# boyden/NuHTC

Measured on AMD Instinct MI355X. Metric: tiles/sec (256x256) whole-node, higher is better.
Workload: dtype f32

## Files before the change

include/nuhtc_hip.h:

```cpp
#ifndef NUHTC_HIP_H
#define NUHTC_HIP_H

#include <stddef.h>
#include <stdint.h>

#ifdef __cplusplus
extern "C" {
#endif

#define NUHTC_ABI_VERSION 12

enum {
  NUHTC_OK = 0,
  NUHTC_E_INVALID = -1,
  NUHTC_E_HIP = -2,
  NUHTC_E_STATE = -3,
  NUHTC_E_CAPACITY = -4,
  NUHTC_E_NOTFOUND = -5
};

enum { NUHTC_CH_AS_IS = 0, NUHTC_CH_SWAP = 1 };

enum { NUHTC_PIPE_BF16_SPLIT = 0, NUHTC_PIPE_FP32 = 1 };

// ... 70 lines not shown
  NUHTC_OVERLAP_POLYGON = 1
};

int nuhtc_merge_overlap(int device, const int32_t* boxes, const float* scores, const int32_t* areas, const uint32_t* bits,
                        const int64_t* bit_off, int64_t n, int64_t n_words, int overlap, double thr, int x_min, int y_min,
                        int x_max, int y_max, uint8_t* keep_dev, void* stream);

int nuhtc_check(nuhtc_engine* e, void* stream);

int nuhtc_get_buffer(nuhtc_engine* e, const char* name, void** dev_ptr, int64_t* shape, int* ndim, int* dtype);

int nuhtc_op_gemm(nuhtc_engine* e, const float* A, const float* W, const float* bias, float* C, int M, int N, int K,
                  int act, void* stream);
int nuhtc_op_gemm_split(nuhtc_engine* e, const float* A, const float* W_dev, const float* W_host, const float* bias, float* C, int M,
                        int N, int K, int act, void* stream);
int nuhtc_op_ln_gemm(nuhtc_engine* e, const float* X_dev, int T, const int* rows_dev, const float* W_host, const float* bias_host, const float* ln_g_host,
                     const float* ln_b_host, float* C_dev, int M, int N, int K, int act, void* stream);
int nuhtc_op_gemm_ln_gemm(nuhtc_engine* e, const float* A_dev, const float* Wp_host, const float* bp_host, const float* res_dev, const int* row_map_dev,
                          const float* W_host, const float* bias_host, const float* ln_g_host, const float* ln_b_host, float* Y_dev, float* C_dev, int M,
                          int Kp, int K, int N, int act, void* stream);
int nuhtc_op_merge_ln_gemm(nuhtc_engine* e, const float* X_dev, int B, int H, int W, int C, const float* W_host, const float* ln_g_host,
                           const float* ln_b_host, float* Y_dev, void* stream);
int nuhtc_op_swin_mlp(nuhtc_engine* e, const float* x_dev, const float* ln_g_dev, const float* ln_b_dev, const float* w1_host,
                      const float* b1_dev, const float* w2_host, const float* b2_dev, float* out_dev, int T, int C, void* stream);
int nuhtc_op_swin_proj_mlp(nuhtc_engine* e, const float* x_dev, const float* att_dev, const float* wp_host, const float* bp_dev,
                           const float* ln_g_dev, const float* ln_b_dev, const float* w1_host, const float* b1_dev, const float* w2_host,
                           const float* b2_dev, float* out_dev, int T, int C, void* stream);
int nuhtc_op_roi_align(nuhtc_engine* e, const float* feat_nhwc, int N, int H, int W, const float* rois, int R, int P,
                       float spatial_scale, int sampling_ratio, float* out, void* stream);
int nuhtc_op_nms(nuhtc_engine* e, const float* boxes, const float* scores, int n, float iou_thr, int32_t* keep_idx,
                 int32_t* count_dev, void* stream);
int nuhtc_op_cc_mask(nuhtc_engine* e, const float* sem_pred_dev, int B, int h, int w, int H, int W, uint8_t* mask_out_dev, void* stream);
int nuhtc_op_cc_proposals(nuhtc_engine* e, const uint8_t* mask_dev, int B, int H, int W, int open, int min_area, int cap, uint8_t* opened_out,
                          uint8_t* filled_out, int32_t* labels_out, int32_t* stats_out, float* boxes_out, int32_t* counts_out,
                          int32_t* overflow_out, void* stream);
typedef struct nuhtc_conv3_args {
  const float* in;
  float* out;
  const float* w;
  const float* bias;
  int32_t nimg, H, W, act;
  const int32_t* nimg_dev;
  int32_t pipe;
  int32_t N2;
  const float* w2;
  const float* b2;
  int32_t act2, store_out;
  float* out2;
  const float* res2;
  float* out3;
  const float* wn1;
  const float* bn1;
  float* outn1;
  int32_t n_more;
  const float* more_in[3];
  float* more_out2[3];
  int32_t more_H[3], more_W[3];
} nuhtc_conv3_args;
int nuhtc_op_conv3(nuhtc_engine* e, const nuhtc_conv3_args* a, void* stream);
enum { NUHTC_ORDER_TOKEN = 0, NUHTC_ORDER_COMPACT = 1 };
typedef struct nuhtc_wmsa_args {
  const float* x;
  float* out;
  const float* ln_g;
  const float* ln_b;
  const float* qkv_w;
  const float* qkv_b;
  const float* rel_table;
  int32_t B, H, W, C;
  int32_t shifted, pipe, out_order;
} nuhtc_wmsa_args;
int nuhtc_op_window_msa(nuhtc_engine* e, const nuhtc_wmsa_args* a, void* stream);
int nuhtc_op_patch_embed(nuhtc_engine* e, const uint8_t* tiles_dev, int B, int th, int tw, int valid_h, int valid_w, float scale_factor, int channel_mode,
                         const float* mean, const float* std, const float* w_host, const float* b_host, const float* ln_g_host, const float* ln_b_host,
                         float* tok_dev, float* img_dev, void* stream);
int nuhtc_op_layernorm(nuhtc_engine* e, const float* x_dev, const float* g_dev, const float* b_dev, float* y_dev, int rows, int C, void* stream);
int nuhtc_op_merge_ln(nuhtc_engine* e, const float* x_dev, const float* g_dev, const float* b_dev, float* y_dev, int B, int H, int W, int C, void* stream);
int nuhtc_op_fpn_lateral(nuhtc_engine* e, const float* X_dev, int B, int H, int W, int C, const float* W_host, const float* bias_host, const float* ln_g_host,
                         const float* ln_b_host, const float* parent_dev, float* out_dev, void* stream);
int nuhtc_op_sem_fuse(nuhtc_engine* e, const float* g0, const float* g1, const float* g2, const float* g3, float* out, int B, int H, int W, void* stream);
int nuhtc_op_pointwise64(nuhtc_engine* e, const float* x_dev, const float* w_dev, const float* b_dev, float* y_dev, int rows, const int32_t* rows_dev,
                         int rows_mul, int sigmoid, void* stream);
int nuhtc_op_fpn_mean_pool(nuhtc_engine* e, const float* const maps[4], const int32_t hw[4], int B, float* feat_dev, void* stream);
typedef struct nuhtc_bbox_tail_args {
  const float* h;
  const float* cls_w;
  const float* cls_b;
  const float* reg_w;
  const float* reg_b;
  int32_t nc, cap, refine;
  float stds[4];
  float img_w, img_h;
  const int32_t* r_dev;
  float* rois;
  float* cls;
  float* reg;
} nuhtc_bbox_tail_args;
int nuhtc_op_bbox_tail(nuhtc_engine* e, const nuhtc_bbox_tail_args* a, void* stream);
typedef struct nuhtc_det_post_args {
  const float* rois;
  const float* cls0;
  const float* cls1;
  const float* cls2;
  const float* reg2;
  const int32_t* roi_off;
  const int32_t* roi_cnt;
  int32_t B, nc, total, cap;
  float stds[4];
  float img_w, img_h, scale, score_thr, nms_iou;
  int32_t max_per_img, limit;
  float* dets;
  int32_t* labels;
  int32_t* counts;
  float* mask_rois;
  int32_t* det_off;
  int32_t* det_total;
  int32_t* cand_count;
  float* cand_scores;
  int32_t* cand_ids;
  float* cand_boxes;
} nuhtc_det_post_args;
int nuhtc_op_det_post(nuhtc_engine* e, const nuhtc_det_post_args* a, void* stream);
typedef struct nuhtc_paste_args {
  const float* prob;
  const float* mask_rois;
  const int32_t* det_off;
  const int32_t* det_counts;
  int32_t B, D, max_keep, H, W, vH, vW;
  float scale, thr;
  uint32_t* masks;
  int32_t* areas;
} nuhtc_paste_args;
int nuhtc_op_paste(nuhtc_engine* e, const nuhtc_paste_args* a, void* stream);
typedef struct nuhtc_tile_post_args {
  const float* dets;
  const int32_t* labels;
  const int32_t* areas;
  const int32_t* det_counts;
  const uint32_t* masks;
  uint8_t* keep;
  int32_t B, max_keep, H, W, vH, vW, margin, min_area;
  float thr;
} nuhtc_tile_post_args;
int nuhtc_op_tile_post(nuhtc_engine* e, const nuhtc_tile_post_args* a, void* stream);
int nuhtc_op_rpn_select(nuhtc_engine* e, const float* const out[4], const int32_t h[4], const int32_t w[4], int B, int nms_pre, int img_h, int img_w,
                        float min_size, float* cand_boxes, float* cand_scores, int32_t* cand_count, void* stream);
int nuhtc_op_nms_levels(nuhtc_engine* e, const float* boxes, const float* scores, const int32_t* group_count, int B, int G, int slot, float iou_thr,
                        int max_keep, int route, float* dets, int32_t* src, int32_t* counts, void* stream);
int nuhtc_op_build_rois(nuhtc_engine* e, const float* cc_boxes, const int32_t* cc_counts, int cc_cap, const float* rpn_dets, const int32_t* rpn_counts,
                        int rpn_cap, const float* fixed, int n_fixed, int B, int cap, float* rois, int32_t* roi_off, int32_t* roi_cnt, int32_t* total,
                        void* stream);

#define NUHTC_AP_AUTO 0
#define NUHTC_AP_GEMM 1
#define NUHTC_AP_KERNEL 2
#define NUHTC_AP_FP16 3
int nuhtc_op_attn_pool(nuhtc_engine* e, const float* F, int B, int HW, float tau, int route, float* G, void* stream);
typedef struct nuhtc_roi_feats_args {
  const float* x0;
  const float* x1;
  const float* sem;
  const float* x0sem;
  const float* G2;
  const float* G3;
  const float* rois;
  const int32_t* r_dev;
// ... 175 lines not shown
```

nuhtc_amd/csrc/common.h:

```cpp
#pragma once
#include <hip/hip_runtime.h>

#include <cstdint>
#include <cstdio>
#include <map>
#include <string>
#include <vector>

#include "../../include/nuhtc_hip.h"

#define WS 7
#define WS2 49
#define HEAD_DIM 32
#define FPN_C 64
#define FC_C 256

struct HostTensor {
  std::vector<float> data;
  std::vector<int64_t> shape;
};

struct BufInfo {
  void* ptr;
  std::vector<int64_t> shape;
  int dtype;
};

struct EngineError {
  int code;
  std::string msg;
};

#define HIP_CHECK(e, expr)                                                                              \
  do {                                                                                                  \
    hipError_t _err = (expr);                                                                           \
    if (_err != hipSuccess) {                                                                           \
      (e)->err = std::string(#expr) + " failed: " + hipGetErrorString(_err) + " at " + __FILE__ + ":" + \
                 std::to_string(__LINE__);                                                              \
      return NUHTC_E_HIP;                                                                               \
    }                                                                                                   \
  } while (0)

#define FAIL(e, code, message) \
  do {                         \
    (e)->err = (message);      \
    return (code);             \
  } while (0)

static inline int cdiv(int a, int b) { return (a + b - 1) / b; }
static inline bool launched() { return hipGetLastError() == hipSuccess; }

class DevScratch {
 public:
  DevScratch() = default;
  DevScratch(const DevScratch&) = delete;
  DevScratch& operator=(const DevScratch&) = delete;
  ~DevScratch() {
    for (void* p : ptrs_) hipFree(p);
  }
  template <typename T = void>
  T* alloc(size_t bytes) {
    void* p = nullptr;
    if (hipMalloc(&p, bytes) != hipSuccess) { ok_ = false; return nullptr; }
    ptrs_.push_back(p);
    return static_cast<T*>(p);
  }
  template <typename T>
  T* upload(const T* host, size_t n) {
    T* d = alloc<T>(n * sizeof(T));
    if (d && hipMemcpy(d, host, n * sizeof(T), hipMemcpyHostToDevice) != hipSuccess) { ok_ = false; return nullptr; }
    return d;
  }
  template <typename T>
  T* upload(const std::vector<T>& v) { return upload(v.data(), v.size()); }
  bool ok() const { return ok_; }

 private:
  std::vector<void*> ptrs_;
  bool ok_ = true;
};

struct ProfScope {
  ProfScope(const char* tag, double flops, double bytes, hipStream_t s);
  ~ProfScope();
  void device_rows(const int* m_dev, int m_mul, int m_cap);
  hipStream_t s_;
  int idx_;
};
bool prof_enabled();
int dev_knob(const char* name, int dflt);
int& dev_knob_ref(const char* name, int dflt);
#define DEV_SKIP(bit)                                    \
  do {                                                   \
    static const int& skip_ = dev_knob_ref("SKIP", 0);   \
    if (skip_ & (bit)) return 0;                         \
  } while (0)

enum AMode { A_PLAIN = 0, A_CONV3 = 1, A_LN = 2  };
enum Act { ACT_NONE = 0, ACT_RELU = 1, ACT_GELU = 2, ACT_COS = 3  };
enum StoreMode { ST_PLAIN = 0, ST_ROWMAP = 1, ST_DECONV2 = 2 };

struct Conv3Fuse {
  int N2;
  const void* w2f;
  const float* bias2;
  float* out2;
  int act2;
  const float* res2;
  float* out3;
  const float* wn1;
  const float* bn1;
  float* outn1;
  int store_out;
  int n_more;
  const float* more_in[3];
  float* more_out2[3];
  int more_H[3], more_W[3];
};
int conv3_pack_fuse(const float* w2_host, int N2, std::vector<unsigned short>& out);

struct GemmParams {
  const float* A;
  const float* W;
  const void* Wsplit;
  const float* bias;
  float* C;
  int M, N, K;
  int lda, ldc;
  const int* m_dev;
  int m_mul;
  int amode;
  const float* ln_part;
  int ln_nparts;
  const int* a_rows;
  int seg_k, seg_rows;
  const int* pad_rows;
  int n_pad;
  const float* pad_val;
  float* stats_out;
  int cH, cW, cC;
  const float* zeros;
  int act;
  float alpha;
  const float* res;
  int ldr;
  const float* up;
  int upH, upW;
  const int* row_map;
  int store;
  const float* cos_ri;
  const float* cos_rj;
  float cos_tau;
  int batch;
  long long sA, sW, sC, sRi, sRj;
  unsigned long long* stamps;
  int row_fastest;
  int throughput;
  const Conv3Fuse* fuse;
};
int launch_gemm(const GemmParams& p, hipStream_t s);
int gemm_make_split(const float* w_host, int N, int K, std::vector<unsigned short>& out);

bool conv3_split_supported(const GemmParams& p);
int launch_conv3_split(const GemmParams& p, hipStream_t s);

bool mlp_supported(int C);
size_t mlp_stream_bytes(int C);
void mlp_pack_stream(const float* w1, const float* w2, int C, std::vector<unsigned short>& out);
size_t proj_stream_bytes(int C);
void proj_pack_stream(const float* w, int C, std::vector<unsigned short>& out);
int launch_swin_mlp(const float* x_in, float* x_out, const float* ln_g, const float* ln_b, const void* wstream, const float* b1, const float* b2,
                    int T, int C, hipStream_t s, const float* att = nullptr, const void* pstream = nullptr, const float* bp = nullptr,
                    float* stats_out = nullptr );

bool lnqkv_supported(int C);
void lnqkv_pack_stream(const float* w, int C, std::vector<unsigned short>& out);
int launch_swin_lnqkv(const float* x, float* qkv, const int* src_tok, const int* dst_row, const int* pad_rows, int n_pad, const float* ln_g, const float* ln_b,
                      const void* wstream, const float* bias, int T, int C, hipStream_t s);

int launch_contours(const uint32_t* masks, const uint8_t* keep, const int32_t* counts, int B, int max_per_img, int H, int W,
                    int cap, int16_t* xy, int32_t* n, hipStream_t s);

struct ExportParams {
  const float* boxes; const int32_t* labels; const int32_t* counts; const uint8_t* keep; const uint32_t* masks;
  const int32_t* contour_n; const int16_t* contour_xy;
  int B, K, words, ccap, cap;
  int32_t* n_out; int64_t* idx; float* boxes_out; int32_t* labels_out; int32_t* cn_out; int16_t* xy_out; uint32_t* words_out;
};
int launch_export_kept(const ExportParams& p, int32_t* pos_scratch, hipStream_t s);
int launch_export_crops(const uint32_t* words, const int32_t* n_dev, int cap, int H, int wpr, int32_t* box, int32_t* area, int32_t* off, int32_t* size_scratch,
                        uint32_t* pool, int pool_cap, hipStream_t s);

void cv_linear_tables(int ssize, int dsize, bool horizontal, std::vector<int>& tab);
int launch_preproc(const uint8_t* tiles, float* img, int B, int th, int tw, int Hn, int Wn, int Hv, int Wv, const int* xtab, const int* ytab, int swap,
                   const float* mean_istd, hipStream_t s);
int launch_patch_embed_tiles(const uint8_t* tiles, int B, int th, int tw, int Hn, int Wn, int Hv, int Wv, const int* xtab, const int* ytab, int swap,
                             const float* mean_istd, const float* w, const float* b, const float* g, const float* beta, float* tok, hipStream_t s);
int launch_layernorm(const float* x, const int* src_map, const float* g, const float* b, float* y, int rows, int C, hipStream_t s);
int launch_ln_stats(const float* x, float* stats, int rows, int C, hipStream_t s);
int launch_layernorm_windows(const float* x, const int* src_map, const int* dst_map, const float* g, const float* b, float* y,
                             float* pad_dst, const float* pad_val, int rows, int C, hipStream_t s);
int launch_merge_ln(const float* x, const float* g, const float* b, float* y, int B, int H, int W, int C, hipStream_t s);
int launch_window_attn(const float* qkv, const float* biasP, const float* maskP, const int* mask_any, const int* out_map, float* out,
                       int nWinTotal, int nWperImg, int C, int nH, int split_pipe , hipStream_t s,
                       const unsigned long long* padbits = nullptr ,
                       int bias_row = 0);

int launch_sem_fuse(const float* g0, const float* g1, const float* g2, const float* g3, float* out, int B, int H, int W,
                    hipStream_t s);
int launch_conv1x1_n1(const float* x, const float* w, const float* b, float* y, int rows, int C, hipStream_t s);
int launch_rownorm_inv(const float* x, float* inv, int rows, int C, hipStream_t s);
int launch_transpose(const float* x, float* y, int batch, int rows, int cols, hipStream_t s);

#define POOL_CHUNK 256
struct PoolLevels { const float* x[4]; int hw[4]; int choff[5]; };
int pool_chunks(const int hw[4], int choff[5]);
int launch_fpn_mean_pool(const PoolLevels& p, int B, double* slab, float* feat, hipStream_t s);

int launch_roi_align(const float* feat, int N, int H, int W, int C, const float* rois, int R, const int* r_dev, int P,
                     float scale, int sr, float* out, int accumulate, hipStream_t s);

const char* nuhtc_tu_probe_conv();
const char* nuhtc_tu_probe_gemm();
const char* nuhtc_tu_probe_mlp();
const char* nuhtc_tu_probe_swin();
```

nuhtc_amd/csrc/dense.hip:

```cpp
#include "common.h"

__device__ __forceinline__ float4 bilin_ac(const float* __restrict__ g, int b, int h, int w, int y, int x, int H, int W, int c4) {
  const float sy = h > 1 ? (float)(h - 1) / (float)(H - 1) : 0.f;
  const float sx = w > 1 ? (float)(w - 1) / (float)(W - 1) : 0.f;
  const float fy = sy * y, fx = sx * x;
  const int y0 = (int)fy, x0 = (int)fx;
  const int y1 = y0 + (y0 < h - 1 ? 1 : 0), x1 = x0 + (x0 < w - 1 ? 1 : 0);
  const float ly = fy - y0, lx = fx - x0, hy = 1.f - ly, hx = 1.f - lx;
  const float4* p = reinterpret_cast<const float4*>(g) + (long long)b * h * w * 16 + c4;
  const float4 v00 = p[(y0 * w + x0) * 16], v01 = p[(y0 * w + x1) * 16], v10 = p[(y1 * w + x0) * 16], v11 = p[(y1 * w + x1) * 16];
  float4 r;
  r.x = hy * (hx * v00.x + lx * v01.x) + ly * (hx * v10.x + lx * v11.x);
  r.y = hy * (hx * v00.y + lx * v01.y) + ly * (hx * v10.y + lx * v11.y);
  r.z = hy * (hx * v00.z + lx * v01.z) + ly * (hx * v10.z + lx * v11.z);
  r.w = hy * (hx * v00.w + lx * v01.w) + ly * (hx * v10.w + lx * v11.w);
  return r;
}

__global__ void sem_fuse_kernel(const float* __restrict__ g0, const float* __restrict__ g1, const float* __restrict__ g2,
                                const float* __restrict__ g3, float* __restrict__ out, int B, int H, int W) {
  long long idx = (long long)blockIdx.x * blockDim.x + threadIdx.x;
  long long total = (long long)B * H * W * 16;
  if (idx >= total) return;
  int c4 = idx & 15;
  long long pix = idx >> 4;
  int x = pix % W, y = (pix / W) % H, b = pix / ((long long)W * H);
  float4 a = reinterpret_cast<const float4*>(g0)[idx];
  float4 r = make_float4(fmaxf(a.x, 0.f), fmaxf(a.y, 0.f), fmaxf(a.z, 0.f), fmaxf(a.w, 0.f));
  const float* gs[3] = {g1, g2, g3};
#pragma unroll
  for (int i = 0; i < 3; ++i) {
    int h = H >> (i + 1), w = W >> (i + 1);
    float4 u = bilin_ac(gs[i], b, h, w, y, x, H, W, c4);
    r.x += fmaxf(u.x, 0.f); r.y += fmaxf(u.y, 0.f); r.z += fmaxf(u.z, 0.f); r.w += fmaxf(u.w, 0.f);
  }
  reinterpret_cast<float4*>(out)[idx] = r;
}

int launch_sem_fuse(const float* g0, const float* g1, const float* g2, const float* g3, float* out, int B, int H, int W,
                    hipStream_t s) {
  ProfScope ps("sem_fuse", 0, 4.0 * 64 * B * H * W * 2.33, s);
  long long total = (long long)B * H * W * 16;
  hipLaunchKernelGGL(sem_fuse_kernel, dim3((unsigned)((total + 255) / 256)), dim3(256), 0, s, g0, g1, g2, g3, out, B, H, W);
  return launched() ? 0 : NUHTC_E_HIP;
}

__global__ void conv1x1_n1_kernel(const float* __restrict__ x, const float* __restrict__ w, const float* __restrict__ b,
                                  float* __restrict__ y, long long rows, const int* __restrict__ rows_dev, int rows_mul, int sigmoid) {
  if (rows_dev) { long long rd = (long long)(*rows_dev) * rows_mul; rows = rd < rows ? rd : rows; }
  const int l = threadIdx.x & 15;
  const float4 ww = reinterpret_cast<const float4*>(w)[l];
  const float bias = b[0];
  const long long stride = ((long long)gridDim.x * blockDim.x) >> 4;
  for (long long row = ((long long)blockIdx.x * blockDim.x + threadIdx.x) >> 4; row < rows; row += stride) {
    const float4 v = reinterpret_cast<const float4*>(x)[row * 16 + l];
    float acc = v.x * ww.x + v.y * ww.y + v.z * ww.z + v.w * ww.w;
    acc += __shfl_xor(acc, 1); acc += __shfl_xor(acc, 2); acc += __shfl_xor(acc, 4); acc += __shfl_xor(acc, 8);
    if (l == 0) {
      const float u = acc + bias;
      y[row] = sigmoid ? 1.0f / (1.0f + expf(-u)) : u;
    }
  }
}

int launch_conv1x1_n1(const float* x, const float* w, const float* b, float* y, int rows, int C, hipStream_t s) {
  if (C != 64) return NUHTC_E_INVALID;
  long long threads = (long long)rows * 16;
  if (rows <= 0) return 0;
  hipLaunchKernelGGL(conv1x1_n1_kernel, dim3((unsigned)((threads + 255) / 256)), dim3(256), 0, s, x, w, b, y, (long long)rows,
                     (const int*)nullptr, 1, 0);
  return launched() ? 0 : NUHTC_E_HIP;
}

int launch_conv1x1_n1_dev(const float* x, const float* w, const float* b, float* y, int rows_cap, const int* rows_dev, int rows_mul,
                          int sigmoid, hipStream_t s) {
  long long threads = (long long)rows_cap * 16;
  if (rows_cap <= 0) return 0;
  const long long nb = (threads + 255) / 256;
  hipLaunchKernelGGL(conv1x1_n1_kernel, dim3((unsigned)(nb < 8192 ? nb : 8192)), dim3(256), 0, s, x, w, b, y, (long long)rows_cap,
                     rows_dev, rows_mul, sigmoid);
  return launched() ? 0 : NUHTC_E_HIP;
}

__global__ void rownorm_inv_kernel(const float* __restrict__ x, float* __restrict__ inv, long long rows) {
  long long row = ((long long)blockIdx.x * blockDim.x + threadIdx.x) >> 4;
  const int l = threadIdx.x & 15;
  float acc = 0.f;
  if (row < rows) {
    float4 v = reinterpret_cast<const float4*>(x)[row * 16 + l];
    acc = v.x * v.x + v.y * v.y + v.z * v.z + v.w * v.w;
  }
  acc += __shfl_xor(acc, 1); acc += __shfl_xor(acc, 2); acc += __shfl_xor(acc, 4); acc += __shfl_xor(acc, 8);
  if (row < rows && l == 0) inv[row] = 1.0f / fmaxf(sqrtf(acc), 1e-8f);
}

int launch_rownorm_inv(const float* x, float* inv, int rows, int C, hipStream_t s) {
  if (C != 64) return NUHTC_E_INVALID;
  long long threads = (long long)rows * 16;
  hipLaunchKernelGGL(rownorm_inv_kernel, dim3((unsigned)((threads + 255) / 256)), dim3(256), 0, s, x, inv, (long long)rows);
  return launched() ? 0 : NUHTC_E_HIP;
}

__global__ void transpose_kernel(const float* __restrict__ x, float* __restrict__ y, int rows, int cols) {
  __shared__ float t[32][33];
  const float* xb = x + (long long)blockIdx.z * rows * cols;
  float* yb = y + (long long)blockIdx.z * rows * cols;
  int c0 = blockIdx.x * 32, r0 = blockIdx.y * 32;
  int tx = threadIdx.x & 31, ty = threadIdx.x >> 5;
  for (int j = ty; j < 32; j += 8) {
    int r = r0 + j, c = c0 + tx;
    t[j][tx] = (r < rows && c < cols) ? xb[(long long)r * cols + c] : 0.f;
  }
  __syncthreads();
  for (int j = ty; j < 32; j += 8) {
    int c = c0 + j, r = r0 + tx;
    if (r < rows && c < cols) yb[(long long)c * rows + r] = t[tx][j];
  }
}

int launch_transpose(const float* x, float* y, int batch, int rows, int cols, hipStream_t s) {
  hipLaunchKernelGGL(transpose_kernel, dim3(cdiv(cols, 32), cdiv(rows, 32), batch), dim3(256), 0, s, x, y, rows, cols);
  return launched() ? 0 : NUHTC_E_HIP;
}
```

nuhtc_amd/csrc/engine.h:

```cpp
#pragma once
#include <unordered_map>

#include "common.h"

struct StageGeom {
  int H, W, C, nH;
  int Hp, Wp, nW;
  int* map[2];
  int* cidx[2];
  int* ctok[2];
  int* vrow[2];
  unsigned long long* padbits[2];
  int* brow;
  int bias_row;
  float* mask;
  int* mask_any;
};

enum BlockRoute { ROUTE_PLAIN, ROUTE_A_LN, ROUTE_FUSED };

struct BlockW {
  BlockRoute route;
  float *n1g, *n1b, *relbT , *qkv_w, *qkv_b, *proj_w, *proj_b, *n2g, *n2b, *f1_w, *f1_b, *f2_w, *f2_b;
  float *qkv_wln, *qkv_bln, *f1_wln, *f1_bln;
  void* qkv_stream;
  void* mlp_stream;
  void* proj_stream;
};

struct nuhtc_engine {
  nuhtc_config cfg;
  int device = 0;
  std::string err;
  std::map<std::string, HostTensor> raw;
  std::map<std::string, std::vector<int64_t>> schema;
  std::map<std::string, BufInfo> bufs;
  std::vector<void*> allocs;
  struct WSplit { const void* planes; int N, K; };
  std::unordered_map<const float*, WSplit> wsplit;
  bool finalized = false;
  bool debug_tokens = false;
  int lastB = 0;
  int Hn = 0, Wn = 0;
  int Hv = 0, Wv = 0;
  int vh = 0, vw = 0;
  int *rs_xtab = nullptr, *rs_ytab = nullptr;

  StageGeom st[4];
  float *pe_w = nullptr, *pe_b = nullptr, *pe_g = nullptr, *pe_beta = nullptr;
  std::vector<BlockW> blocks[4];
  bool merge_one_launch[3] = {}, out_ln_folded = false, conv_fuse = false;
  float *on_g[4], *on_b[4], *mg_g[3], *mg_b[3], *mg_w[3];
  float *mg_wln[3] = {}, *mg_bln[3] = {};
  int* mg_src[3] = {};
  float *lat_w[4], *lat_b[4], *fpn_w[4], *fpn_b[4];
  float *rpn_w, *rpn_b, *rpn_hw, *rpn_hb;
  void *rpn_hf, *sem_lf[4], *sem_ef;
  float *sem_lw[4], *sem_lb[4], *sem_cw[4], *sem_cb[4], *sem_ew, *sem_eb, *sem_gw, *sem_gb;
  float *fc1_w[3], *fc1_b[3], *fc2_w[3], *fc2_b[3], *head_w[3], *head_b[3];
  float *mk_w[4], *mk_b[4], *mk_up_w, *mk_up_b, *mk_lw, *mk_lb;

  float *img, *tokA, *tokB, *xw, *qkv, *att, *hid;
  float* tok[4] = {};
  float* ln_out[4] = {};
  float *lat_wln[4] = {}, *lat_bln[4] = {};
  const uint8_t* in_tiles = nullptr;
  int in_swap = 0;
  int last_batch = 0;
  float* ln_part2 = nullptr;
  float* ln_part = nullptr;
  float *c[4], *lat[4], *x[4], *rpn[4], *semg[4];
  float *tmpA, *tmpB, *tmpR, *sem_feat, *sem_pred, *x0sem;
  PoolLevels pool{};
  double* pool_slab = nullptr;
  int roi_cap = 0;
  int cand_cap = 0;
  int* overflow = nullptr;
  int* overflow_host = nullptr;
  int32_t* export_pos = nullptr;
  int32_t* crop_size = nullptr;
  hipStream_t own = nullptr;
  hipStream_t side = nullptr;
  hipEvent_t ev_rpn = nullptr, ev_side = nullptr, ev_fpn = nullptr;
  hipStream_t side2 = nullptr;
  hipEvent_t ev_side2 = nullptr;
  struct RoiWs* rw = nullptr;
};

int dev_alloc(nuhtc_engine* e, void** p, size_t bytes);
int upload_bytes(nuhtc_engine* e, void** dst, const void* host, size_t bytes);
template <typename T>
int upload(nuhtc_engine* e, T** dst, const std::vector<T>& v) {
  return upload_bytes(e, (void**)dst, v.data(), v.size() * sizeof(T));
}
template <typename T>
int ws(nuhtc_engine* e, T** p, const char* name, std::vector<int64_t> shape, int dtype) {
  size_t n = 1;
  for (auto d : shape) n *= (size_t)d;
  int rc = dev_alloc(e, (void**)p, n * sizeof(T));
  if (rc) return rc;
  if (name) e->bufs[name] = BufInfo{(void*)*p, shape, dtype};
  return 0;
}
const HostTensor* raw(nuhtc_engine* e, const std::string& name, std::initializer_list<int64_t> shape);
#define RAW(var, name, ...)                                 \
  const HostTensor* var = raw(e, (name), {__VA_ARGS__});    \
  if (!var) return NUHTC_E_STATE;
std::vector<float> pack_conv3(const HostTensor& w, int O, int I);
int upload_gemm_weight(nuhtc_engine* e, float** dst, const std::vector<float>& v, int N, int K);

GemmParams gp(const float* A, const float* W, const float* bias, float* C, int M, int N, int K);
#define RUN(expr)                                                                                        \
  do {                                                                                                   \
    int _rc = (expr);                                                                                    \
    if (_rc) { e->err = std::string(#expr) + " failed (" + std::to_string(_rc) + ")"; return _rc; }     \
  } while (0)
inline int op_finish(nuhtc_engine* e, int rc, hipStream_t s, const char* launch_err, const char* kernel_err) {
  const hipError_t he = hipStreamSynchronize(s);
  if (rc) FAIL(e, rc, launch_err);
  if (he != hipSuccess) FAIL(e, NUHTC_E_HIP, kernel_err);
  return 0;
}
int egemm(nuhtc_engine* e, GemmParams p, hipStream_t s);
int finalize_roi(nuhtc_engine* e);
int alloc_roi_workspace(nuhtc_engine* e);
int run_roi_path(nuhtc_engine* e, int B, const float* rois_fixed, int n_rois, int n_dets, hipStream_t s, const nuhtc_dets* out);
int run_backbone(nuhtc_engine* e, int B, hipStream_t s);
int run_neck_heads(nuhtc_engine* e, int B, hipStream_t s);
int run_fpn(nuhtc_engine* e, int B, hipStream_t s, bool sem_lateral);
int launch_conv1x1_n1_dev(const float* x, const float* w, const float* b, float* y, int rows_cap, const int* rows_dev, int rows_mul,
                          int sigmoid, hipStream_t s);
```

nuhtc_amd/csrc/engine.hip:

```cpp
#include <cmath>
#include <cstdlib>
#include <cstring>
#include <mutex>

#include "common.h"
#include "engine.h"

static const int DEPTHS[4] = {2, 2, 6, 2};
static const int NHEADS[4] = {3, 6, 12, 24};

static thread_local std::string g_create_error;

void nuhtc_default_config(nuhtc_config* c) {
  memset(c, 0, sizeof(*c));
  c->abi_version = NUHTC_ABI_VERSION;
  c->num_classes = 5;
  c->tile_h = c->tile_w = 256;
  c->max_batch = 16;
  c->scale_factor = 2.0f;
  const float mean[3] = {123.675f, 116.28f, 103.53f}, std[3] = {58.395f, 57.12f, 57.375f};
  for (int i = 0; i < 3; ++i) { c->mean[i] = mean[i]; c->std[i] = std[i]; }
  c->rpn_nms_pre = 3000; c->rpn_max_per_img = 1000; c->rpn_nms_iou = 0.7f; c->rpn_min_bbox_size = 10.f;
  c->score_thr = 0.35f; c->nms_iou = 0.5f; c->max_per_img = 500; c->mask_thr_binary = 0.5f;
  c->att_thres = 0.965926f;
// ... 1203 lines not shown
  hipStream_t s = (hipStream_t)stream;
  float mi[6];
  norm_consts(mean, std, mi);
  DevScratch sc;
  const int *xtab = sc.upload(rg.tx), *ytab = sc.upload(rg.ty);
  const float *w = sc.upload(pack_patch_embed(w_host)), *b = sc.upload(b_host, 96), *g = sc.upload(ln_g_host, 96), *beta = sc.upload(ln_b_host, 96);
  if (!sc.ok()) FAIL(e, NUHTC_E_HIP, "patch_embed op: scratch upload failed");
  const int swap = channel_mode == NUHTC_CH_SWAP;
  int rc = launch_patch_embed_tiles(tiles_dev, B, th, tw, rg.Hn, rg.Wn, rg.Hv, rg.Wv, xtab, ytab, swap, mi, w, b, g, beta, tok_dev, s);
  if (!rc && img_dev) rc = launch_preproc(tiles_dev, img_dev, B, th, tw, rg.Hn, rg.Wn, rg.Hv, rg.Wv, xtab, ytab, swap, mi, s);
  return op_finish(e, rc, s, "patch_embed launch failed", "patch_embed kernels failed");
}

int nuhtc_op_layernorm(nuhtc_engine* e, const float* x_dev, const float* g_dev, const float* b_dev, float* y_dev, int rows, int C, void* stream) {
  if (!e || !x_dev || !g_dev || !b_dev || !y_dev) return NUHTC_E_INVALID;
  if (rows < 1 || (C != 96 && C != 192 && C != 384 && C != 768) || (long long)rows * C >= (1ll << 31)) FAIL(e, NUHTC_E_INVALID, "layernorm op: rows >= 1, C in {96, 192, 384, 768}");
  HIP_CHECK(e, hipSetDevice(e->device));
  hipStream_t s = (hipStream_t)stream;
  const int rc = launch_layernorm(x_dev, nullptr, g_dev, b_dev, y_dev, rows, C, s);
  return op_finish(e, rc, s, "layernorm launch failed", "layernorm kernel failed");
}

int nuhtc_op_merge_ln(nuhtc_engine* e, const float* x_dev, const float* g_dev, const float* b_dev, float* y_dev, int B, int H, int W, int C, void* stream) {
  if (!e || !x_dev || !g_dev || !b_dev || !y_dev) return NUHTC_E_INVALID;
  if (B < 1 || H < 2 || W < 2 || (H & 1) || (W & 1)) FAIL(e, NUHTC_E_INVALID, "merge_ln op: H and W must be even (the network input is a multiple of 32)");
  if ((C != 96 && C != 192 && C != 384) || (long long)B * H * W * C >= (1ll << 31)) FAIL(e, NUHTC_E_INVALID, "merge_ln op: C in {96, 192, 384}");
  HIP_CHECK(e, hipSetDevice(e->device));
  hipStream_t s = (hipStream_t)stream;
  const int rc = launch_merge_ln(x_dev, g_dev, b_dev, y_dev, B, H, W, C, s);
  return op_finish(e, rc, s, "merge_ln launch failed", "merge_ln kernel failed");
}

int nuhtc_op_fpn_lateral(nuhtc_engine* e, const float* X_dev, int B, int H, int W, int C, const float* W_host, const float* bias_host, const float* ln_g_host,
                         const float* ln_b_host, const float* parent_dev, float* out_dev, void* stream) {
  if (!e || !X_dev || !W_host || !bias_host || !out_dev || (ln_g_host == nullptr) != (ln_b_host == nullptr)) return NUHTC_E_INVALID;
  if (B < 1 || H < 1 || W < 1 || (C != 96 && C != 192 && C != 384 && C != 768) || (long long)B * H * W * C >= (1ll << 31)) FAIL(e, NUHTC_E_INVALID, "fpn_lateral op: size out of range");
  if (parent_dev && ((H & 1) || (W & 1))) FAIL(e, NUHTC_E_INVALID, "fpn_lateral op: a map with a parent has even sides");
  HIP_CHECK(e, hipSetDevice(e->device));
  hipStream_t s = (hipStream_t)stream;
  const int T = B * H * W;
  DevScratch sc;
  GemmParams p;
  int rc = 0;
  if (ln_g_host) {
    std::vector<float> wl, bl;
    fold_ln(W_host, bias_host, ln_g_host, ln_b_host, 64, C, wl, bl);
    std::vector<unsigned short> split;
    if ((rc = gemm_make_split(wl.data(), 64, C, split))) FAIL(e, rc, "gemm_make_split failed");
    float* st = sc.alloc<float>((size_t)T * (C / 96) * 2 * sizeof(float));
    p = lateral_params(X_dev, sc.upload(wl), sc.upload(bl), out_dev, B, H, W, C, st, parent_dev);
    p.Wsplit = sc.upload(split);
    if (!sc.ok()) FAIL(e, NUHTC_E_HIP, "fpn_lateral op: scratch upload failed");
    rc = launch_ln_stats(X_dev, st, T * (C / 96), 96, s);
  } else {
    p = lateral_params(X_dev, sc.upload(W_host, (size_t)64 * C), sc.upload(bias_host, 64), out_dev, B, H, W, C, nullptr, parent_dev);
    if (!sc.ok()) FAIL(e, NUHTC_E_HIP, "fpn_lateral op: scratch upload failed");
  }
  if (!rc) rc = launch_gemm(p, s);
  return op_finish(e, rc, s, "fpn_lateral launch failed", "fpn_lateral kernels failed");
}

int nuhtc_op_sem_fuse(nuhtc_engine* e, const float* g0, const float* g1, const float* g2, const float* g3, float* out, int B, int H, int W, void* stream) {
  if (!e || !g0 || !g1 || !g2 || !g3 || !out) return NUHTC_E_INVALID;
  if (B < 1 || H < 8 || W < 8 || H % 8 || W % 8 || (long long)B * H * W * 64 >= (1ll << 31)) FAIL(e, NUHTC_E_INVALID, "sem_fuse op: H and W must be multiples of 8 (level 0 of a network input that is a multiple of 32)");
  HIP_CHECK(e, hipSetDevice(e->device));
  hipStream_t s = (hipStream_t)stream;
  const int rc = launch_sem_fuse(g0, g1, g2, g3, out, B, H, W, s);
  return op_finish(e, rc, s, "sem_fuse launch failed", "sem_fuse kernel failed");
}

int nuhtc_op_pointwise64(nuhtc_engine* e, const float* x_dev, const float* w_dev, const float* b_dev, float* y_dev, int rows, const int32_t* rows_dev,
                         int rows_mul, int sigmoid, void* stream) {
  if (!e || !x_dev || !w_dev || !b_dev || !y_dev) return NUHTC_E_INVALID;
  if (rows < 1 || (long long)rows * 64 >= (1ll << 31)) FAIL(e, NUHTC_E_INVALID, "pointwise64 op: rows out of range");
  if (!rows_dev && sigmoid) FAIL(e, NUHTC_E_INVALID, "pointwise64 op: the fixed-row form has no sigmoid");
  if (rows_dev && rows_mul < 1) FAIL(e, NUHTC_E_INVALID, "pointwise64 op: rows_mul must be >= 1");
  HIP_CHECK(e, hipSetDevice(e->device));
  hipStream_t s = (hipStream_t)stream;
  const int rc = rows_dev ? launch_conv1x1_n1_dev(x_dev, w_dev, b_dev, y_dev, rows, rows_dev, rows_mul, sigmoid ? 1 : 0, s)
                          : launch_conv1x1_n1(x_dev, w_dev, b_dev, y_dev, rows, 64, s);
  return op_finish(e, rc, s, "pointwise64 launch failed", "pointwise64 kernel failed");
}

int nuhtc_op_fpn_mean_pool(nuhtc_engine* e, const float* const maps[4], const int32_t hw[4], int B, float* feat_dev, void* stream) {
  if (!e || !maps || !hw || !feat_dev || B < 1) return NUHTC_E_INVALID;
  PoolLevels p{};
  int hwi[4];
  for (int l = 0; l < 4; ++l) {
    if (!maps[l] || hw[l] < 1 || (long long)B * hw[l] * 64 >= (1ll << 31)) FAIL(e, NUHTC_E_INVALID, "fpn_mean_pool op: null or empty level");
    hwi[l] = hw[l];
    p.x[l] = maps[l];
  }
  int rc = pool_layout(hwi, p);
  if (rc) FAIL(e, rc, "pool_chunks: empty FPN level");
  HIP_CHECK(e, hipSetDevice(e->device));
  hipStream_t s = (hipStream_t)stream;
  DevScratch sc;
  double* slab = sc.alloc<double>(pool_slab_bytes(p, B));
  if (!sc.ok()) FAIL(e, NUHTC_E_HIP, "fpn_mean_pool op: scratch allocation failed");
  rc = launch_fpn_mean_pool(p, B, slab, feat_dev, s);
  return op_finish(e, rc, s, "fpn_mean_pool launch failed", "fpn_mean_pool kernels failed");
}

#ifdef NUHTC_DEV
extern "C" int nuhtc_dev_realloc(nuhtc_engine* e, int which, unsigned long long* addr) {
  if (!e || which < 0 || which > 5) return NUHTC_E_INVALID;
  HIP_CHECK(e, hipSetDevice(e->device));
  HIP_CHECK(e, hipDeviceSynchronize());
  float** slots[6] = {&e->tokA, &e->tokB, &e->xw, &e->qkv, &e->att, &e->hid};
  void* base = nullptr;
  size_t bytes = 0;
  HIP_CHECK(e, hipMemGetAddressRange((hipDeviceptr_t*)&base, &bytes, (hipDeviceptr_t)*slots[which]));
  void* p = nullptr;
  HIP_CHECK(e, hipMalloc(&p, bytes));
  HIP_CHECK(e, hipMemset(p, 0, bytes));
  e->allocs.push_back(p);
  *slots[which] = (float*)p;
  if (which == 0) e->bufs["tokens"].ptr = p;
  e->tok[0] = e->tokA; e->tok[1] = e->tokB;
  if (addr) *addr = (unsigned long long)p;
  return 0;
}
#endif
```

nuhtc_amd/csrc/gemm.hip:

```cpp
#include <cstdlib>
#include <cstring>
#include <map>
#include <mutex>
#include <vector>
#include <cstdio>

#include "common.h"

#include "split_math.h"

template <int MT, int NT, int WM, int WN>
__device__ __forceinline__ void gemm_epilogue(const GemmParams& p, f32x16 (&acc)[MT][NT], float* lds, float* __restrict__ C, int z, int m0, int n0,
                                              int Meff, const float* ln_rstd = nullptr ) {
  const int tid = threadIdx.x;
  const int lane = tid & 63, wave = tid >> 6;
  const int wm = wave / WN, wn = wave % WN;
  const int i32 = lane & 31, half = lane >> 5;
  const float* ri = p.cos_ri ? p.cos_ri + (long long)z * p.sRi : nullptr;
  const float* rj = p.cos_rj ? p.cos_rj + (long long)z * p.sRj : nullptr;
  __syncthreads();
  float* tb = lds + wave * (32 * 32);
  const int rr = lane >> 3, c4 = (lane & 7) * 4;
#pragma unroll
  for (int mi = 0; mi < MT; ++mi) {
    int mrow[4], drow[4], aux[4];
    unsigned okmask = 0;
#pragma unroll
    for (int j = 0; j < 4; ++j) {
      const int m = m0 + (wm * MT + mi) * 32 + 8 * j + rr;
      if (m < Meff) okmask |= 1u << j;
      mrow[j] = m < Meff ? m : Meff - 1;
      drow[j] = mrow[j];
      aux[j] = 0;
    }
    if (p.store == ST_ROWMAP) {
      int d[4];
#pragma unroll
      for (int j = 0; j < 4; ++j) d[j] = p.row_map[mrow[j]];
#pragma unroll
      for (int j = 0; j < 4; ++j) { if (d[j] < 0) okmask &= ~(1u << j); drow[j] = d[j] >= 0 ? d[j] : 0; }
    }
    if (p.up) {
#pragma unroll
      for (int j = 0; j < 4; ++j) {
        const int hw = p.upH * p.upW;
        const int b = mrow[j] / hw, q = mrow[j] - b * hw;
        const int y = q / p.upW, x = q - y * p.upW;
        aux[j] = (b * (p.upH >> 1) + (y >> 1)) * (p.upW >> 1) + (x >> 1);
      }
    } else if (p.store == ST_DECONV2) {
#pragma unroll
      for (int j = 0; j < 4; ++j) {
        const int hw = p.cH * p.cW;
        const int b = mrow[j] / hw, q = mrow[j] - b * hw;
        const int y = q / p.cW, x = q - y * p.cW;
        aux[j] = (b * (2 * p.cH) + 2 * y) * (2 * p.cW) + 2 * x;
      }
    }
    float riv[4];
    if (p.act == ACT_COS) {
#pragma unroll
      for (int j = 0; j < 4; ++j) riv[j] = ri[mrow[j]];
    }
    float lnr[4] = {1.f, 1.f, 1.f, 1.f};
    if (ln_rstd) {
#pragma unroll
      for (int j = 0; j < 4; ++j) lnr[j] = ln_rstd[(wm * MT + mi) * 32 + 8 * j + rr];
    }
    float s_piv[4] = {0.f, 0.f, 0.f, 0.f}, s_1[4] = {0.f, 0.f, 0.f, 0.f}, s_2[4] = {0.f, 0.f, 0.f, 0.f};
    const float* colp = p.act == ACT_COS ? rj : p.bias;
    const float* rowp = p.res ? p.res : p.up;
    const int rowld = p.res ? p.ldr : p.N;
    unsigned rowoff[4];
#pragma unroll
    for (int j = 0; j < 4; ++j) rowoff[j] = (unsigned)(p.res ? drow[j] : aux[j]) * (unsigned)rowld + (unsigned)(n0 + wn * NT * 32 + c4);
    v4f colv[NT];
#pragma unroll
    for (int t = 0; t < NT; ++t) {
      colv[t] = v4f{0.f, 0.f, 0.f, 0.f};
      if (colp) colv[t] = *reinterpret_cast<const v4f*>(colp + n0 + (wn * NT + t) * 32 + c4);
    }
    v4f rowv[4];
#define EPI_LOADS(t_)                                                                                                   \
  if (rowp) {                                                                                                           \
    _Pragma("unroll") for (int j = 0; j < 4; ++j)                                                                       \
        rowv[j] = *reinterpret_cast<const v4f*>(rowp + rowoff[j] + (t_) * 32);                                          \
  }
    EPI_LOADS(0)
#pragma unroll
    for (int t = 0; t < NT; ++t) {
#pragma unroll
      for (int r = 0; r < 16; ++r) tb[((r & 3) + 8 * (r >> 2) + 4 * half) * 32 + i32] = acc[mi][t][r];
      const int n = n0 + (wn * NT + t) * 32 + c4;
      v4f v[4];
#pragma unroll
      for (int j = 0; j < 4; ++j) {
        v[j] = *reinterpret_cast<const v4f*>(tb + (8 * j + rr) * 32 + c4) * p.alpha;
        if (ln_rstd) v[j] *= lnr[j];
        if (p.bias) v[j] += colv[t];
        if (p.act == ACT_RELU) {
          v[j].x = fmaxf(v[j].x, 0.f); v[j].y = fmaxf(v[j].y, 0.f); v[j].z = fmaxf(v[j].z, 0.f); v[j].w = fmaxf(v[j].w, 0.f);
        } else if (p.act == ACT_GELU) {
          v[j].x = gelu_erf(v[j].x); v[j].y = gelu_erf(v[j].y); v[j].z = gelu_erf(v[j].z); v[j].w = gelu_erf(v[j].w);
        } else if (p.act == ACT_COS) {
          v[j].x = fmaxf(v[j].x * riv[j] * colv[t].x - p.cos_tau, 0.f) + p.cos_tau;
          v[j].y = fmaxf(v[j].y * riv[j] * colv[t].y - p.cos_tau, 0.f) + p.cos_tau;
          v[j].z = fmaxf(v[j].z * riv[j] * colv[t].z - p.cos_tau, 0.f) + p.cos_tau;
          v[j].w = fmaxf(v[j].w * riv[j] * colv[t].w - p.cos_tau, 0.f) + p.cos_tau;
        }
        if (rowp) v[j] += rowv[j];
      }
      if (p.stats_out) {
#pragma unroll
        for (int j = 0; j < 4; ++j) {
          if (t == 0) s_piv[j] = __shfl(v[j].x, lane & ~7);
          const v4f d = v[j] - s_piv[j];
          s_1[j] += (d.x + d.y) + (d.z + d.w);
          s_2[j] = fmaf(d.x, d.x, fmaf(d.y, d.y, fmaf(d.z, d.z, fmaf(d.w, d.w, s_2[j]))));
        }
      }
      __builtin_amdgcn_sched_barrier(0);
      if (t + 1 < NT) EPI_LOADS(t + 1)
      __builtin_amdgcn_sched_barrier(0);
#ifdef NUHTC_GEMM_NOSTORE
#ifndef NUHTC_GEMM_NOSTORE_K
#define NUHTC_GEMM_NOSTORE_K 0
#endif
      if (p.alpha == 12345.f || (NUHTC_GEMM_NOSTORE_K && p.K != NUHTC_GEMM_NOSTORE_K))
#endif
#pragma unroll
      for (int j = 0; j < 4; ++j) {
        if (!((okmask >> j) & 1u)) continue;
        if (p.store == ST_DECONV2) {
          const int tap = n / p.ldc, oc = n - tap * p.ldc;
          *reinterpret_cast<v4f*>(C + ((long long)aux[j] + (tap >> 1) * (2 * p.cW) + (tap & 1)) * p.ldc + oc) = v[j];
        } else {
          *reinterpret_cast<v4f*>(C + (long long)drow[j] * p.ldc + n) = v[j];
        }
      }
      __builtin_amdgcn_sched_barrier(0);
    }
    if (p.stats_out) {
      constexpr float inv_n = 1.0f / (32.0f * NT * WN);
      const int ntn = p.N / (32 * NT * WN), tile_n = n0 / (32 * NT * WN);
#pragma unroll
      for (int j = 0; j < 4; ++j) {
#pragma unroll
        for (int o = 1; o < 8; o <<= 1) { s_1[j] += __shfl_xor(s_1[j], o); s_2[j] += __shfl_xor(s_2[j], o); }
        if ((lane & 7) == 0 && ((okmask >> j) & 1u)) {
          const float dm = s_1[j] * inv_n;
          *reinterpret_cast<float2*>(p.stats_out + ((long long)drow[j] * ntn + tile_n) * 2) = make_float2(s_piv[j] + dm, fmaxf(s_2[j] - s_1[j] * dm, 0.f));
        }
      }
    }
#undef EPI_LOADS
  }
}

template <int MT, int NT, int WM, int WN, int BK, int AMODE>
__global__ __launch_bounds__(256, (MT * NT <= 3 ? 4 : 3)) void gemm_kernel(GemmParams p) {
  static_assert(WM * WN == 4, "4 waves per block");
  constexpr int BM = 32 * MT * WM, BN = 32 * NT * WN;
  constexpr int KC = BK / 4;
  constexpr int RPP = 256 / KC;
  constexpr int NA = (BM + RPP - 1) / RPP, NB = (BN + RPP - 1) / RPP;
  constexpr int LDK = BK + 4;
  constexpr int KH = BK / 2;
  __shared__ __attribute__((aligned(16))) float lds[2 * LDK * (BM + BN)];
  float* As = lds;
  float* Bs = lds + 2 * LDK * BM;

  const int tid = threadIdx.x;
  const int lane = tid & 63, wave = tid >> 6;
  const int wm = wave / WN, wn = wave % WN;
  const int i32 = lane & 31, half = lane >> 5;
  const int nTilesN = p.N / BN;
  const int xcd = blockIdx.x & 7, slot = blockIdx.x >> 3;
  const int tile_m = (slot / nTilesN) * 8 + xcd, tile_n = slot % nTilesN;
  const int m0 = tile_m * BM, n0 = tile_n * BN;
  const int z = blockIdx.z;

  int Meff = p.M;
  if (p.m_dev) {
    int md = *p.m_dev * p.m_mul;
    Meff = md < Meff ? md : Meff;
  }
  if (m0 >= Meff) return;

#ifdef NUHTC_GEMM_STAMPS
  unsigned long long st0 = __builtin_amdgcn_s_memtime(), st1 = 0, st2 = 0, st3 = 0, st5 = 0, st6 = 0;
#define STAMP(x_) x_
#else
#define STAMP(x_)
#endif
  const float* __restrict__ A = p.A + (long long)z * p.sA;
  const float* __restrict__ Wt = p.W + (long long)z * p.sW;
  float* __restrict__ C = p.C + (long long)z * p.sC;

  const int kc = tid % KC;
  const int rbase = tid / KC;
  const float* a_ptr[NA];
  unsigned a_ok[NA];
#pragma unroll
  for (int j = 0; j < NA; ++j) {
    int r = rbase + RPP * j;
    r = r < BM ? r : BM - 1;
    int m = m0 + r;
    m = m < Meff ? m : Meff - 1;
    if (AMODE == A_PLAIN) {
      a_ptr[j] = A + (long long)m * p.lda + kc * 4;
      a_ok[j] = 0;
    } else {
      const int hw = p.cH * p.cW;
      const int rr = m - (m / hw) * hw;
      const int y = rr / p.cW, x = rr - y * p.cW;
      unsigned bits = 0;
#pragma unroll
      for (int t = 0; t < 9; ++t) {
        const int yy = y + t / 3 - 1, xx = x + t % 3 - 1;
        if (yy >= 0 && yy < p.cH && xx >= 0 && xx < p.cW) bits |= 1u << t;
      }
      a_ok[j] = bits;
      a_ptr[j] = A + (long long)m * p.cC + kc * 4;
    }
  }
// ... 85 lines not shown
    }                                                                                                          \
  }
#define READ_FRAGS(buf_, q_, FA_, FB_) { _Pragma("unroll") for (int f = 0; f < NRD; ++f) READ_ONE(f, buf_, q_, FA_, FB_) }
#define MFMA_AT(i_, FA_, FB_)                                                                                  \
  {                                                                                                            \
    const int e = (i_) / (MT * NT), mi = ((i_) % (MT * NT)) / NT, t = (i_) % NT;                               \
    acc[mi][t] = __builtin_amdgcn_mfma_f32_32x32x2f32(FA_[mi][e], FB_[t][e], acc[mi][t], 0, 0, 0);             \
  }
#define MFMA_GROUP(FA_, FB_) { _Pragma("unroll") for (int i = 0; i < NMF; ++i) MFMA_AT(i, FA_, FB_) }

  const int nk = p.K / BK;
  LOAD_TILE(0)
  STORE_TILE(0)
  __syncthreads();
  LOAD_TILE(nk > 1 ? 1 : 0)
  READ_FRAGS(0, 0, fa_a, fa_b)
  STAMP(__builtin_amdgcn_s_waitcnt(0xC07F); st1 = __builtin_amdgcn_s_memtime();)
  int kt = 0;
#define KT_BODY(LD_)                                                                                           \
  {                                                                                                            \
    const int buf = kt & 1;                                                                                    \
    _Pragma("unroll") for (int i = 0; i < NMF; ++i) {                                                          \
      MFMA_AT(i, fa_a, fa_b)                                                                                   \
      __builtin_amdgcn_sched_barrier(0);                                                                       \
      _Pragma("unroll") for (int u = 0; u < FPG; ++u) {                                                        \
        const int f = i * FPG + u;                                                                             \
        STAMP(if (f == NRD) { unsigned long long w0 = __builtin_amdgcn_s_memtime(); __builtin_amdgcn_s_waitcnt(0x0070); st6 += __builtin_amdgcn_s_memtime() - w0; }) \
        if (f < NRD) READ_ONE(f, buf, 1, fb_a, fb_b)                                                           \
        else STORE_ONE(f - NRD, buf ^ 1)   \
      }                                                                                                        \
      __builtin_amdgcn_sched_barrier(0);                                                                       \
    }                                                                                                          \
    __builtin_amdgcn_s_waitcnt(0xC07F);                    \
    STAMP(st5 -= __builtin_amdgcn_s_memtime();)                                                                \
    __builtin_amdgcn_s_barrier();             \
    STAMP(st5 += __builtin_amdgcn_s_memtime();)                                                                \
    __builtin_amdgcn_sched_barrier(0);                                                                         \
    if (LD_) CONV_BEGIN()                                                                                      \
    _Pragma("unroll") for (int i = 0; i < NMF; ++i) {                                                          \
      MFMA_AT(i, fb_a, fb_b)                                                                                   \
      __builtin_amdgcn_sched_barrier(0);                                                                       \
      _Pragma("unroll") for (int u = 0; u < FPG; ++u) {                                                        \
        const int f = i * FPG + u;                                                                             \
        if (f < NST) { if (LD_) LOAD_ONE(f, kt + 2) }                                                          \
        else READ_ONE(f - NST, buf ^ 1, 0, fa_a, fa_b)                                                         \
      }                                                                                                        \
      __builtin_amdgcn_sched_barrier(0);                                                                       \
    }                                                                                                          \
    if (LD_) CONV_END()                                                                                        \
  }
  for (; kt + 2 < nk; ++kt) KT_BODY(1)
  KT_BODY(0)
  ++kt;
#undef KT_BODY
  READ_FRAGS(kt & 1, 1, fb_a, fb_b)
  MFMA_GROUP(fa_a, fa_b)
  MFMA_GROUP(fb_a, fb_b)
#undef CONV_BEGIN
#undef CONV_END
#undef LOAD_ONE
#undef STORE_ONE
#undef LOAD_TILE
#undef STORE_TILE
#undef READ_ONE
#undef READ_FRAGS
#undef MFMA_AT
#undef MFMA_GROUP

  STAMP(st2 = __builtin_amdgcn_s_memtime();)
  gemm_epilogue<MT, NT, WM, WN>(p, acc, lds, C, z, m0, n0, Meff);
#ifdef NUHTC_GEMM_STAMPS
  st3 = __builtin_amdgcn_s_memtime();
  __builtin_amdgcn_s_waitcnt(0x0070);
  if (lane == 0 && p.stamps) {
    unsigned hw;
    asm volatile("s_getreg_b32 %0, hwreg(HW_REG_HW_ID)" : "=s"(hw));
    unsigned long long* o = p.stamps + ((long long)blockIdx.x * 4 + wave) * 8;
    o[0] = st0; o[1] = st1; o[2] = st2; o[3] = st3; o[4] = __builtin_amdgcn_s_memtime(); o[5] = hw; o[6] = st5; o[7] = st6;
  }
#endif
#undef STAMP
}

template <int MT, int NT, int AMODE>
__global__ __launch_bounds__(256, (MT * NT <= 4 ? 3 : 2)) void gemm_split_kernel(GemmParams p) {
  constexpr int WM = 4, WN = 1, BK = 16;
  constexpr int BM = 128 * MT, BN = 32 * NT;
  constexpr int KC = BK / 4, RPP = 256 / KC, NA = BM / RPP;
  constexpr int LDK = BK + 4;
  constexpr int BP = 28;
  constexpr int NCH = BN * 6, NB = (NCH + 255) / 256;
  constexpr int LDSF = 2 * (LDK * BM + BP * BN) > 4 * 32 * 32 ? 2 * (LDK * BM + BP * BN) : 4 * 32 * 32;
  __shared__ __attribute__((aligned(16))) float lds[LDSF + (AMODE == A_LN ? 2 * BM : 0)];
  float* As = lds;
  float* Bs = lds + 2 * LDK * BM;
  const int tid = threadIdx.x;
  const int lane = tid & 63, wave = tid >> 6;
  const int i32 = lane & 31, half = lane >> 5;
  const int nTilesN = p.N / BN;
  int bid = blockIdx.x;
  if (AMODE == A_LN && p.n_pad > 0) {
    const int pad_blocks = ((p.n_pad + 63) / 64 + 7) / 8 * 8;
    if (bid < pad_blocks) {
      const int r0 = bid * 64 + wave * 16;
      const v4f* src = reinterpret_cast<const v4f*>(p.pad_val);
      for (int r = r0; r < r0 + 16 && r < p.n_pad; ++r) {
        v4f* dst = reinterpret_cast<v4f*>(p.C + (long long)p.pad_rows[r] * p.ldc);
        for (int c = lane; c < p.N / 4; c += 64) dst[c] = src[c];
      }
      return;
    }
    bid -= pad_blocks;
  }
  const int xcd = bid & 7, slot = bid >> 3;
  const int rowTilesPerXcd = ((p.M + BM - 1) / BM + 7) / 8;
  const int tile_m = p.row_fastest ? (slot % rowTilesPerXcd) * 8 + xcd : (slot / nTilesN) * 8 + xcd;
  const int tile_n = p.row_fastest ? slot / rowTilesPerXcd : slot % nTilesN;
  const int m0 = tile_m * BM, n0 = tile_n * BN;
  const int z = blockIdx.z;
  int Meff = p.M;
  if (p.m_dev) {
    int md = *p.m_dev * p.m_mul;
    Meff = md < Meff ? md : Meff;
  }
  if (m0 >= Meff) return;
#ifdef NUHTC_GEMM_STAMPS
  unsigned long long st0 = __builtin_amdgcn_s_memtime(), st1 = 0, st2 = 0, st3 = 0, st5 = 0, st6 = 0;
  const unsigned long long rt0 = __builtin_amdgcn_s_memrealtime();
#define STAMP(x_) x_
#else
#define STAMP(x_)
#endif
  const float* __restrict__ A = p.A + (long long)z * p.sA;
  float* __restrict__ C = p.C + (long long)z * p.sC;
  const char* __restrict__ Wsp = reinterpret_cast<const char*>(p.Wsplit);

  static_assert(KC == 4 && RPP == 64, "staging lane map below assumes BK = 16");
  const int kc = tid & 3, rbase = ((tid >> 5) << 3) + (((tid >> 2) & 1) << 2) + ((tid >> 3) & 3);
  const float* a_ptr[NA];
  unsigned a_ok[NA];
  float a_mean[NA];
#pragma unroll
  for (int j = 0; j < NA; ++j) {
    int m = m0 + rbase + RPP * j;
    m = m < Meff ? m : Meff - 1;
    a_mean[j] = 0.f;
    if (AMODE == A_PLAIN) {
      a_ptr[j] = A + (long long)m * p.lda + kc * 4;
      a_ok[j] = 0;
    } else if (AMODE == A_LN) {
      const long long src = p.a_rows ? p.a_rows[m] : m;
      a_ptr[j] = A + src * p.lda + kc * 4;
      a_ok[j] = 0;
    } else {
      const int hw = p.cH * p.cW;
      const int rr = m - (m / hw) * hw;
      const int y = rr / p.cW, x = rr - y * p.cW;
      unsigned bits = 0;
#pragma unroll
      for (int t = 0; t < 9; ++t) {
        const int yy = y + t / 3 - 1, xx = x + t % 3 - 1;
        if (yy >= 0 && yy < p.cH && xx >= 0 && xx < p.cW) bits |= 1u << t;
      }
      a_ok[j] = bits;
      a_ptr[j] = A + (long long)m * p.cC + kc * 4;
    }
  }
// ... 146 lines not shown
      float2 q[16];
      float msum = 0.f, m2 = 0.f;
#pragma unroll
      for (int t = 0; t < 16; ++t) if (t < p.ln_nparts) q[t] = pp[t + (t >= half_parts ? second : 0)];
#pragma unroll
      for (int t = 0; t < 16; ++t) if (t < p.ln_nparts) { msum += q[t].x; m2 += q[t].y; }
      const float mean = msum / (float)p.ln_nparts;
      float dev = 0.f;
#pragma unroll
      for (int t = 0; t < 16; ++t) if (t < p.ln_nparts) { const float d = q[t].x - mean; dev = fmaf(d, d, dev); }
      m2 = fmaf((float)(p.K / p.ln_nparts), dev, m2);
      lds[LDSF + tid] = 1.0f / sqrtf(m2 / (float)p.K + 1e-5f);
      lds[LDSF + BM + tid] = mean;
    }
    __syncthreads();
#pragma unroll
    for (int j = 0; j < NA; ++j) a_mean[j] = lds[LDSF + BM + rbase + RPP * j];
  }
  S_STORE_TILE(0)
  __syncthreads();
  if (nk > 1) S_LOAD_TILE(1)
#pragma unroll
  for (int h = 0; h < 2 * MT; ++h) S_READ_A(h, 0)
#pragma unroll
  for (int t = 0; t < NT; ++t) S_READ_B(t, 0)
#pragma unroll
  for (int u = 0; u < NSP; ++u) S_SPLIT_PAIR(u, pc)
  int kt = 0;
  STAMP(__builtin_amdgcn_s_waitcnt(0xC07F); st1 = __builtin_amdgcn_s_memtime();)
#define S_BODY(HN, HN2)                                                                                        \
  {                                                                                                            \
    const int buf = kt & 1;                                                                                    \
    if (HN2) S_CONV_BEGIN()                                                                                    \
    _Pragma("unroll") for (int i = 0; i < PB; ++i) {                                                           \
      S_MFMA(i)                                                                                                \
      __builtin_amdgcn_sched_barrier(0);                                                                       \
      _Pragma("unroll") for (int u = 0; u < FPA; ++u) {                                                        \
        const int f = i * FPA + u;                                                                             \
        STAMP(if (f == 0 && HN) { unsigned long long w0 = __builtin_amdgcn_s_memtime(); __builtin_amdgcn_s_waitcnt(0x0070); st6 += __builtin_amdgcn_s_memtime() - w0; }) \
        if (f < NST) { if (HN) S_STORE_ONE(f, buf ^ 1) }                                                       \
        else if (f < NUA) { if (HN2) S_LOAD_ONE(f - NST, kt + 2) }                                             \
      }                                                                                                        \
      __builtin_amdgcn_sched_barrier(0);                                                                       \
    }                                                                                                          \
    if (HN2) S_CONV_END()                                                                                      \
    __builtin_amdgcn_s_waitcnt(0xC07F);                    \
    STAMP(st5 -= __builtin_amdgcn_s_memtime();)                                                                \
    __builtin_amdgcn_s_barrier();                                                                              \
    STAMP(st5 += __builtin_amdgcn_s_memtime();)                                                                \
    __builtin_amdgcn_sched_barrier(0);                                                                         \
    if (HN) { _Pragma("unroll") for (int h = 0; h < 2 * MT; ++h) S_READ_A(h, buf ^ 1) }                        \
    if (HN) { _Pragma("unroll") for (int t = 0; t < NT; ++t) if (TM * t + TM <= PB) S_READ_B(t, buf ^ 1) }    \
    __builtin_amdgcn_sched_barrier(0);                                                                         \
    _Pragma("unroll") for (int i = PB; i < NMF; ++i) {                                                         \
      S_MFMA(i)                                                                                                \
      __builtin_amdgcn_sched_barrier(0);                                                                       \
      _Pragma("unroll") for (int u = 0; u < FPB; ++u) {                                                        \
        const int f = (i - PB) * FPB + u - SOFF;                                                               \
        if (f >= 0 && f < NSP) { if (HN) S_SPLIT_PAIR(f, pn) }                                                 \
      }                                                                                                        \
      if (HN && i % TM == TM - 1 && i / TM * TM + TM > PB) S_READ_B(i / TM, buf ^ 1)    \
      __builtin_amdgcn_sched_barrier(0);                                                                       \
    }                                                                                                          \
    if (HN) { _Pragma("unroll") for (int mi = 0; mi < MT; ++mi) { pc[mi][0] = pn[mi][0]; pc[mi][1] = pn[mi][1]; pc[mi][2] = pn[mi][2]; } } \
  }
  for (; kt + 2 < nk; ++kt) S_BODY(1, 1)
  if (kt + 1 < nk) { S_BODY(1, 0) ++kt; }
  S_BODY(0, 0)
#undef S_BODY
#undef S_MFMA
#undef S_CONV_BEGIN
#undef S_CONV_END
#undef S_LOAD_ONE
#undef S_STORE_ONE
#undef S_SPLIT_PAIR
#undef S_SPLIT_BODY
#undef S_READ_A
#undef S_READ_B
  __syncthreads();
#undef S_LOAD_TILE
#undef S_AOFF
#undef S_STORE_TILE
  STAMP(st2 = __builtin_amdgcn_s_memtime();)
  gemm_epilogue<MT, NT, WM, WN>(p, acc, lds, C, z, m0, n0, Meff, AMODE == A_LN ? lds + LDSF : nullptr);
#ifdef NUHTC_GEMM_STAMPS
  st3 = __builtin_amdgcn_s_memtime();
  __builtin_amdgcn_s_waitcnt(0x0070);
  if (lane == 0 && p.stamps) {
    unsigned hw;
    asm volatile("s_getreg_b32 %0, hwreg(HW_REG_HW_ID)" : "=s"(hw));
    unsigned long long* o = p.stamps + ((long long)blockIdx.x * 4 + wave) * 8;
    o[0] = st0; o[1] = st1; o[2] = st2; o[3] = st3; o[4] = __builtin_amdgcn_s_memtime(); o[5] = hw; o[6] = st5;
    o[7] = __builtin_amdgcn_s_memrealtime() - rt0;
  }
#endif
#undef STAMP
}

template <int MT, int NT, int WM, int WN>
static void launch_cfg(const GemmParams& q, int mtiles, hipStream_t s) {
  constexpr int BN = 32 * NT * WN;
  dim3 grid(cdiv(mtiles, 8) * 8 * (q.N / BN), 1, q.batch > 0 ? q.batch : 1);
  if (q.amode == A_CONV3) hipLaunchKernelGGL((gemm_kernel<MT, NT, WM, WN, 16, A_CONV3>), grid, dim3(256), 0, s, q);
  else hipLaunchKernelGGL((gemm_kernel<MT, NT, WM, WN, 16, A_PLAIN>), grid, dim3(256), 0, s, q);
}

static const float* zero_page() {
  static std::map<int, float*> pages;
  static std::mutex mu;
  std::lock_guard<std::mutex> lock(mu);
  int dev = 0;
  if (hipGetDevice(&dev) != hipSuccess) return nullptr;
  auto it = pages.find(dev);
  if (it != pages.end()) return it->second;
  float* z = nullptr;
  if (hipMalloc(&z, 256) != hipSuccess || hipMemset(z, 0, 256) != hipSuccess || hipDeviceSynchronize() != hipSuccess) return nullptr;
  pages[dev] = z;
  return z;
}

int gemm_make_split(const float* w_host, int N, int K, std::vector<unsigned short>& out) {
  if (!w_host || N <= 0 || K <= 0 || K % 8) return NUHTC_E_INVALID;
  out.assign((size_t)N * K * 3, 0);
  for (int n = 0; n < N; ++n)
    for (int k = 0; k < K; ++k)
      bf16_split3(w_host[(size_t)n * K + k], out.data() + (((size_t)n * (K / 8) + k / 8) * 3) * 8 + (k & 7), 8);
  return 0;
}

template <int MT, int NT>
static void launch_split(const GemmParams& q, hipStream_t s) {
  const int mtiles = cdiv(q.M, 128 * MT);
  dim3 grid(cdiv(mtiles, 8) * 8 * (q.N / (32 * NT)), 1, q.batch > 0 ? q.batch : 1);
  if (q.amode == A_LN && q.n_pad > 0) grid.x += cdiv(cdiv(q.n_pad, 64), 8) * 8;
  static const int& lds_pad = dev_knob_ref("GEMM_LDS_PAD", 0);
  const unsigned pad = (unsigned)lds_pad;
  if (q.amode == A_CONV3) hipLaunchKernelGGL((gemm_split_kernel<MT, NT, A_CONV3>), grid, dim3(256), pad, s, q);
  else if (q.amode == A_LN) {
    if constexpr (NT == 3 || (NT == 2 && MT == 1)) hipLaunchKernelGGL((gemm_split_kernel<MT, NT, A_LN>), grid, dim3(256), pad, s, q);
  } else hipLaunchKernelGGL((gemm_split_kernel<MT, NT, A_PLAIN>), grid, dim3(256), pad, s, q);
}

int launch_gemm(const GemmParams& p, hipStream_t s) {
  if (p.M <= 0) return 0;
  if (p.K % 32 != 0 || p.N % 32 != 0) return NUHTC_E_INVALID;
  if (p.amode == A_CONV3 && (p.cC % 32 != 0 || p.K != 9 * p.cC)) return NUHTC_E_INVALID;
  if ((p.res && p.up) || (p.act == ACT_COS && p.bias)) return NUHTC_E_INVALID;
  if ((p.amode == A_LN) != (p.ln_part != nullptr) ||
      (p.amode == A_LN && (!p.Wsplit || (p.N % 96 != 0 && p.N != 64) || p.batch > 1 || p.ln_nparts < 1 || p.ln_nparts > 16 || p.K % p.ln_nparts != 0 ||
                           (p.seg_k && (p.K != 2 * p.seg_k || p.seg_k % 16 != 0 || p.ln_nparts % 4 != 0 || !p.a_rows || p.seg_rows < 1)) || (p.n_pad > 0 && (!p.pad_rows || !p.pad_val)))))
    return NUHTC_E_INVALID;
  if (p.stats_out && (!p.Wsplit || p.N % 96 != 0 || p.batch > 1 || (p.store != ST_PLAIN && p.store != ST_ROWMAP) || p.amode == A_CONV3)) return NUHTC_E_INVALID;
  if ((p.res && (long long)p.M * p.ldr >= (1ll << 31)) || (p.up && (long long)p.M * p.N >= (1ll << 31))) return NUHTC_E_INVALID;
  GemmParams q = p;
  if (q.alpha == 0.f) q.alpha = 1.f;
  if (q.Wsplit && q.batch > 1) q.Wsplit = nullptr;
  int nt = (p.N % 96 == 0) ? 3 : (p.N % 128 == 0) ? 4 : (p.N % 64 == 0) ? 2 : 1;
  {
    static const int& fill = dev_knob_ref("GEMM_FILL", 500);
    static const int& sfill = dev_knob_ref("SPLIT_FILL", 256);
    static const int& force_nt = dev_knob_ref("SPLIT_NT", 0);
    long long mt = cdiv(p.M, 128) * (long long)(p.batch > 0 ? p.batch : 1);
    if (p.m_dev) mt = (mt + 1) / 2;
    const int limit = q.Wsplit ? sfill : fill;
    if (!(q.Wsplit && nt == 3) && q.amode != A_LN)
      while (nt > 1 && mt * (p.N / (32 * nt)) < limit) { if (nt > 2 && p.N % 64 == 0) nt = 2; else nt = 1; }
    if (force_nt > 0 && p.N % (32 * force_nt) == 0) nt = force_nt;
    if (q.amode == A_LN && nt != 3 && nt != 2) return NUHTC_E_INVALID;
    if (q.stats_out && nt != 3) return NUHTC_E_INVALID;
  }
  if (q.amode == A_CONV3 && !q.zeros) {
    q.zeros = zero_page();
    if (!q.zeros) return NUHTC_E_HIP;
  }
  const bool halo = conv3_split_supported(q);
  if (p.fuse && !halo) return NUHTC_E_INVALID;
  const double nb = p.batch > 0 ? p.batch : 1;
  const char* tag = "gemm";
  if (prof_enabled()) {
    static std::map<long long, std::string> names;
    long long key = ((long long)nt << 40) | ((long long)p.N << 20) | p.K | ((long long)(p.amode == A_CONV3) << 44) | ((long long)halo << 45) | ((long long)(p.fuse ? p.fuse->N2 / 32 : 0) << 46) | ((long long)(p.fuse ? p.fuse->n_more : 0) << 52) |
                    ((long long)(p.amode == A_LN) << 50) | ((long long)(p.stats_out != nullptr) << 51);
    auto it = names.find(key);
    if (it == names.end())
      it = names.emplace(key, "gemm_kernel<" + std::to_string(nt) + ">|N" + std::to_string(p.N) + "|K" + std::to_string(p.K) + (p.amode == A_CONV3 ? (halo ? "|conv3halo" : "|conv3") : "") + (p.fuse ? "+pw" + std::to_string(p.fuse->N2) + (p.fuse->n_more ? "x" + std::to_string(1 + p.fuse->n_more) + "maps" : "") : "") +
                                    (p.amode == A_LN ? "|ln" : "") + (p.stats_out ? "|stats" : "")).first;
    tag = it->second.c_str();
  }
  const double row_term = p.res ? (double)p.M * p.N : p.up ? 0.25 * p.M * p.N : 0.0;
  const double fuse_flop = p.fuse ? 2.0 * p.M * 64 * (p.fuse->N2 + (p.fuse->outn1 ? 1 : 0)) : 0.0;
  const double fuse_bytes = p.fuse ? 4.0 * p.M * (p.fuse->N2 * (p.fuse->out3 ? 3.0 : 1.0) + (p.fuse->outn1 ? 1 : 0) - (p.fuse->store_out ? 0 : p.N)) : 0.0;
  double more_rows = 0.0;
  if (p.fuse && p.fuse->n_more > 0 && p.amode == A_CONV3)
    for (int k = 0; k < p.fuse->n_more && k < 3; ++k) more_rows += (double)(p.M / (p.cH * p.cW)) * p.fuse->more_H[k] * p.fuse->more_W[k];
  const double more_flop = p.fuse ? 2.0 * more_rows * 64 * (p.K + p.fuse->N2) : 0.0, more_bytes = p.fuse ? 4.0 * more_rows * (64 + p.fuse->N2) : 0.0;
  ProfScope ps(tag, 2.0 * p.M * p.N * p.K * nb + fuse_flop + more_flop, 4.0 * nb * ((double)p.M * p.K + (double)p.N * p.K + (double)p.M * p.N + row_term) + fuse_bytes + more_bytes, s);
  ps.device_rows(p.m_dev, p.m_mul, p.M);
#ifdef NUHTC_GEMM_STAMPS
  static unsigned long long* stamp_buf = nullptr;
  if (!stamp_buf && hipMalloc(&stamp_buf, 8ull * 8 * 4 * 65536) != hipSuccess) return NUHTC_E_HIP;
  q.stamps = stamp_buf;
#endif
  if (q.Wsplit && !halo && q.amode != A_CONV3 && !q.m_dev) {
    static const int& order_knob = dev_knob_ref("SPLIT_ROW_FASTEST", -1);
    const double w_bytes = 6.0 * q.N * q.K, a_xcd_bytes = 4.0 * ((double)q.M / 8.0) * q.K;
    q.row_fastest = order_knob >= 0 ? order_knob : (w_bytes > 6.0e6 && a_xcd_bytes < 3.0e6);
  }
  if (halo) {
    const int rc = launch_conv3_split(q, s);
    if (rc) return rc;
  } else if (q.Wsplit) {
    static const int& force_mt = dev_knob_ref("SPLIT_MT", 0);
    const long long blocks2 = (long long)cdiv(p.M, 256) * (p.N / (32 * nt));
    const bool mt2 = force_mt ? force_mt == 2 : (!p.m_dev && nt == 3 && (p.throughput || (blocks2 >= 512 && p.M >= 131072)));
    if (mt2 && nt == 3) launch_split<2, 3>(q, s);
    else if (nt == 1) launch_split<1, 1>(q, s);
    else if (nt == 2) launch_split<1, 2>(q, s);
    else if (nt == 3) launch_split<1, 3>(q, s);
    else if (nt == 6) launch_split<1, 6>(q, s);
    else launch_split<1, 4>(q, s);
  } else if (nt == 1) launch_cfg<1, 1, 4, 1>(q, cdiv(p.M, 128), s);
  else if (nt == 2) launch_cfg<1, 2, 4, 1>(q, cdiv(p.M, 128), s);
  else if (nt == 3) launch_cfg<1, 3, 4, 1>(q, cdiv(p.M, 128), s);
  else launch_cfg<1, 4, 4, 1>(q, cdiv(p.M, 128), s);
#ifdef NUHTC_GEMM_STAMPS
  {
    static int cnt = 0, dump_at = -1;
    if (dump_at < 0) { const char* e = getenv("NUHTC_STAMP_AT"); dump_at = e ? atoi(e) : 5; }
    if (++cnt == dump_at) {
      hipDeviceSynchronize();
      int nb_ = cdiv(cdiv(p.M, 128), 8) * 8 * (p.N / (32 * nt));
      if (nb_ > 65536) nb_ = 65536;
      std::vector<unsigned long long> h((size_t)nb_ * 32);
      hipMemcpy(h.data(), stamp_buf, h.size() * 8, hipMemcpyDeviceToHost);
      FILE* f = fopen("/tmp/stamps.txt", "w");
      for (int b = 0; b < nb_; ++b) for (int w = 0; w < 4; ++w) { auto* o = &h[((size_t)b * 4 + w) * 8]; fprintf(f, "%d %d %llu %llu %llu %llu %llu %llu %llu %llu\n", b, w, o[0], o[1], o[2], o[3], o[4], o[5], o[6], o[7]); }
      fclose(f);
    }
  }
#endif
  return launched() ? 0 : NUHTC_E_HIP;
}

const char* nuhtc_tu_probe_gemm() {
#ifdef NUHTC_GEMM_NOSTORE
  return "NUHTC_GEMM_NOSTORE";
#elif defined(NUHTC_GEMM_PROBE_NOSPLIT)
  return "NUHTC_GEMM_PROBE_NOSPLIT";
#else
  return nullptr;
#endif
}
```

nuhtc_amd/csrc/roi_engine.hip:

```cpp
#include <cmath>
#include <cstring>

#include "engine.h"
#include "proposals.h"
#include "roi.h"

#define BIG_SPLIT_MAX 512
struct RoiWs {
  float *cand_boxes, *cand_scores;
  unsigned* rpn_keys;
  int rpn_key_stride;
  int* cand_count;
  float *nms_sboxes;
  int *nms_src, *nms_ntotal, *nms_seg_start, *nms_seg_n, *nms_pos;
  unsigned long long* nms_keepbits;
  unsigned long long* nms_mask;
  float* rpn_dets;
  int *rpn_src, *rpn_counts;
  int rpn_slot, rpn_cap, rpn_pow2;
  unsigned char *cc_a, *cc_b, *cc_touch;
  int *cc_labels, *cc_stats, *cc_counts, *cc_list, *cc_nlist;
  float* cc_boxes;
  float* rois;
  int *roi_off, *roi_cnt, *roi_total;
  float *G2, *G3, *ap_inv, *ap_S, *ap_Ft;
  float *feats, *h1, *h2;
  int *fb_count, *fb_list, *mid_list;
  float* big_part;
  unsigned char* fb_flag;
  float *cls[3], *reg[3];
  int total_cap;
  float *dc_boxes, *dc_scores;
  int *dc_ids, *dc_count;
  int det_cap, det_pow2;
  float* det_dets;
  int *det_src, *det_counts, *det_labels;
  float* mask_rois;
  int *det_off, *det_total;
  float *mfeat, *mtmpA, *mtmpB, *mup, *mprob;
  int mask_cap;
  unsigned* masks_own;
  int* areas_own;
  unsigned char* keep_own;
};

static void pack_bbox_head(const float* wc, const float* bc, const float* wr, const float* br, int nc, std::vector<float>& hw, std::vector<float>& hb) {
  hw.assign((size_t)(nc + 6) * 256, 0.f);
  hb.assign(nc + 6, 0.f);
  for (int n = 0; n < nc + 2; ++n) {
    float ss = 0.f;
    for (int k2 = 0; k2 < 256; ++k2) ss += wc[n * 256 + k2] * wc[n * 256 + k2];
    float den = sqrtf(ss) + 1e-6f;
    for (int k2 = 0; k2 < 256; ++k2) hw[n * 256 + k2] = wc[n * 256 + k2] / den;
    hb[n] = bc[n];
  }
  for (int n = 0; n < 4; ++n) {
    for (int k2 = 0; k2 < 256; ++k2) hw[(nc + 2 + n) * 256 + k2] = wr[n * 256 + k2];
    hb[nc + 2 + n] = br[n];
  }
}
static double mask_nms_thr(float thr) { return std::round((double)thr * 1e6) / 1e6; }

int finalize_roi(nuhtc_engine* e) {
  const int nc = e->cfg.num_classes;
  int rc;
  for (int k = 0; k < 3; ++k) {
    const std::string p = "roi_head.bbox_head." + std::to_string(k) + ".";
    RAW(w1, p + "shared_fcs.0.weight", 256, 3136); RAW(b1, p + "shared_fcs.0.bias", 256);
    RAW(w2, p + "shared_fcs.1.weight", 256, 256); RAW(b2, p + "shared_fcs.1.bias", 256);
    RAW(wc, p + "fc_cls.weight", nc + 2, 256); RAW(bc, p + "fc_cls.bias", nc + 2);
    RAW(wr, p + "fc_reg.weight", 4, 256); RAW(br, p + "fc_reg.bias", 4);
    std::vector<float> w1p((size_t)256 * 3136);
    for (int n = 0; n < 256; ++n)
      for (int c = 0; c < 64; ++c)
        for (int bin = 0; bin < 49; ++bin) w1p[(size_t)n * 3136 + bin * 64 + c] = w1->data[(size_t)n * 3136 + c * 49 + bin];
    std::vector<float> hw, hb;
    pack_bbox_head(wc->data.data(), bc->data.data(), wr->data.data(), br->data.data(), nc, hw, hb);
    if ((rc = upload_gemm_weight(e, &e->fc1_w[k], w1p, 256, 3136)) || (rc = upload(e, &e->fc1_b[k], b1->data)) || (rc = upload_gemm_weight(e, &e->fc2_w[k], w2->data, 256, 256)) ||
        (rc = upload(e, &e->fc2_b[k], b2->data)) || (rc = upload(e, &e->head_w[k], hw)) || (rc = upload(e, &e->head_b[k], hb)))
      return rc;
  }
  {
    const std::string p = "roi_head.mask_head.0.";
    for (int j = 0; j < 4; ++j) {
      RAW(w, p + "convs." + std::to_string(j) + ".conv.weight", 64, 64, 3, 3);
      RAW(b, p + "convs." + std::to_string(j) + ".conv.bias", 64);
      if ((rc = upload_gemm_weight(e, &e->mk_w[j], pack_conv3(*w, 64, 64), 64, 576)) || (rc = upload(e, &e->mk_b[j], b->data))) return rc;
    }
    RAW(uw, p + "upsample.weight", 64, 64, 2, 2); RAW(ub, p + "upsample.bias", 64);
    RAW(lw, p + "conv_logits.weight", 1, 64, 1, 1); RAW(lb, p + "conv_logits.bias", 1);
    std::vector<float> w((size_t)256 * 64), b(256);
    for (int ic = 0; ic < 64; ++ic)
      for (int oc = 0; oc < 64; ++oc)
        for (int t = 0; t < 4; ++t) w[((size_t)t * 64 + oc) * 64 + ic] = uw->data[((size_t)ic * 64 + oc) * 4 + t];
    for (int t = 0; t < 4; ++t)
      for (int oc = 0; oc < 64; ++oc) b[t * 64 + oc] = ub->data[oc];
    if ((rc = upload_gemm_weight(e, &e->mk_up_w, w, 256, 64)) || (rc = upload(e, &e->mk_up_b, b)) || (rc = upload(e, &e->mk_lw, lw->data)) || (rc = upload(e, &e->mk_lb, lb->data))) return rc;
  }
  return 0;
}

static int round_up(int v, int m) { return (v + m - 1) / m * m; }
static int pow2_ge(int v) { int p = 2; while (p < v) p <<= 1; return p; }

int alloc_roi_workspace(nuhtc_engine* e) {
  const nuhtc_config& c = e->cfg;
  const int B = c.max_batch;
  const int Hn = e->Hn, Wn = e->Wn;
  RoiWs* w = new RoiWs();
  memset(w, 0, sizeof(*w));
  e->rw = w;
  int rc;
  if ((rc = nms_set_attributes())) { e->err = "hipFuncSetAttribute(nms_prepare) failed"; return rc; }
  w->rpn_slot = c.rpn_nms_pre;
  int maxc = 0;
  for (int l = 0; l < 4; ++l) maxc += std::min(c.rpn_nms_pre, e->st[l].H * e->st[l].W * 3);
  w->rpn_cap = round_up(std::max(maxc, 64), 64) + 64 * 3;
  w->rpn_pow2 = pow2_ge(maxc);
  e->roi_cap = c.max_cc_proposals + c.rpn_max_per_img;
  w->det_cap = round_up(e->roi_cap * c.num_classes, 64);
  w->det_pow2 = pow2_ge(e->roi_cap * c.num_classes);
  if (maxc > NMS_MAX_CAP || w->det_cap > NMS_MAX_CAP) { e->err = "candidate capacity exceeds NMS_MAX_CAP (reduce rpn_nms_pre / max_cc_proposals)"; return NUHTC_E_INVALID; }
  const int nmscap = std::max(w->rpn_cap, w->det_cap);
  w->rpn_key_stride = round_up(e->st[0].H * e->st[0].W * 3, 64);
  if ((rc = ws(e, &w->rpn_keys, nullptr, {B, 4, w->rpn_key_stride}, 1)) ||
      (rc = ws(e, &w->cand_boxes, "rpn_cand_boxes", {B, 4, w->rpn_slot, 4}, 0)) || (rc = ws(e, &w->cand_scores, "rpn_cand_scores", {B, 4, w->rpn_slot}, 0)) ||
      (rc = ws(e, &w->cand_count, "rpn_cand_count", {B, 4}, 1)) || (rc = ws(e, &w->nms_sboxes, nullptr, {B, nmscap, 4}, 0)) ||
      (rc = ws(e, &w->nms_src, nullptr, {B, nmscap}, 1)) || (rc = ws(e, &w->nms_ntotal, nullptr, {B}, 1)) ||
      (rc = ws(e, &w->nms_seg_start, nullptr, {B, 4}, 1)) || (rc = ws(e, &w->nms_seg_n, nullptr, {B, 4}, 1)) ||
      (rc = ws(e, &w->nms_pos, nullptr, {B, nmscap}, 1)) || (rc = ws(e, &w->nms_keepbits, nullptr, {B, nmscap / 64}, 3)) ||
      (rc = ws(e, &w->nms_mask, nullptr, {B, nmscap, nmscap / 64}, 3)) || (rc = ws(e, &w->rpn_dets, "rpn_props", {B, c.rpn_max_per_img, 5}, 0)) ||
      (rc = ws(e, &w->rpn_src, nullptr, {B, c.rpn_max_per_img}, 1)) || (rc = ws(e, &w->rpn_counts, "rpn_counts", {B}, 1)))
    return rc;
  const int64_t HW = (int64_t)Hn * Wn;
  const int ccc = std::max(c.max_cc_proposals, 1);
  if ((rc = ws(e, &w->cc_a, nullptr, {B, HW}, 2)) || (rc = ws(e, &w->cc_b, "cc_mask", {B, Hn, Wn}, 2)) || (rc = ws(e, &w->cc_touch, nullptr, {B, HW}, 2)) ||
      (rc = ws(e, &w->cc_labels, "cc_labels", {B, Hn, Wn}, 1)) || (rc = ws(e, &w->cc_stats, nullptr, {B, HW, 5}, 1)) ||
      (rc = ws(e, &w->cc_list, nullptr, {B, CC_LIST_CAP}, 1)) || (rc = ws(e, &w->cc_nlist, nullptr, {B}, 1)) ||
      (rc = ws(e, &w->cc_boxes, "cc_props", {B, ccc, 4}, 0)) || (rc = ws(e, &w->cc_counts, "cc_counts", {B}, 1)) ||
      (rc = ws(e, &e->overflow, nullptr, {4}, 1)))
    return rc;
  w->total_cap = B * e->roi_cap;
  const int T = w->total_cap;
  if ((rc = ws(e, &w->rois, "rois", {T, 5}, 0)) || (rc = ws(e, &w->roi_off, "roi_off", {B}, 1)) || (rc = ws(e, &w->roi_cnt, "roi_counts", {B}, 1)) ||
      (rc = ws(e, &w->roi_total, "roi_total", {1}, 1)) || (rc = ws(e, &w->G2, "G2", {B, e->st[2].H * e->st[2].W, 64}, 0)) ||
      (rc = ws(e, &w->G3, "G3", {B, e->st[3].H * e->st[3].W, 64}, 0)) || (rc = ws(e, &w->feats, "bbox_feats", {T, 49, 64}, 0)) ||
      (rc = ws(e, &w->h1, nullptr, {T, 256}, 0)) || (rc = ws(e, &w->h2, "h2", {T, 256}, 0)) ||
      (rc = ws(e, &w->ap_inv, nullptr, {B, e->st[2].H * e->st[2].W}, 0)) ||
      (rc = ws(e, &w->ap_S, nullptr, {B, (int64_t)e->st[2].H * e->st[2].W, (int64_t)e->st[2].H * e->st[2].W}, 0)) ||
      (rc = ws(e, &w->ap_Ft, nullptr, {B, 64, e->st[2].H * e->st[2].W}, 0)) ||
      (rc = ws(e, &w->fb_count, "roi_fallback_count", {8}, 1)) || (rc = ws(e, &w->mid_list, nullptr, {T}, 1)) || (rc = ws(e, &w->fb_list, nullptr, {T}, 1)) || (rc = ws(e, &w->fb_flag, nullptr, {T}, 2)))
    return rc;
  if ((rc = ws(e, &w->big_part, nullptr, {BIG_SPLIT_MAX, 3, 49, 64}, 0))) return rc;
  for (int k = 0; k < 3; ++k) {
    std::string n = std::to_string(k);
    if ((rc = ws(e, &w->cls[k], ("cls" + n).c_str(), {T, 16}, 0)) || (rc = ws(e, &w->reg[k], ("reg" + n).c_str(), {T, 4}, 0))) return rc;
    std::string rn = "rois_stage" + n;
    float* snap;
    if ((rc = ws(e, &snap, rn.c_str(), {T, 5}, 0))) return rc;
  }
  if ((rc = ws(e, &w->dc_boxes, nullptr, {B, w->det_cap, 4}, 0)) || (rc = ws(e, &w->dc_scores, nullptr, {B, w->det_cap}, 0)) ||
      (rc = ws(e, &w->dc_ids, nullptr, {B, w->det_cap}, 1)) || (rc = ws(e, &w->dc_count, "det_cand_count", {B}, 1)) ||
      (rc = ws(e, &w->det_src, nullptr, {B, c.max_per_img}, 1)) || (rc = ws(e, &w->det_counts, nullptr, {B}, 1)))
    return rc;
  w->mask_cap = B * c.max_per_img;
  const int D = w->mask_cap;
  if ((rc = ws(e, &w->mask_rois, "mask_rois", {D, 5}, 0)) || (rc = ws(e, &w->det_off, "det_off", {B}, 1)) || (rc = ws(e, &w->det_total, "det_total", {1}, 1)) ||
      (rc = ws(e, &w->mfeat, "mask_feats", {D, 196, 64}, 0)) || (rc = ws(e, &w->mtmpA, nullptr, {D, 196, 64}, 0)) || (rc = ws(e, &w->mtmpB, nullptr, {D, 196, 64}, 0)) ||
      (rc = ws(e, &w->mup, nullptr, {D, 784, 64}, 0)) || (rc = ws(e, &w->mprob, "mask_prob", {D, 28, 28}, 0)))
    return rc;
  if (hipMemset(e->overflow, 0, 16) != hipSuccess) { e->err = "hipMemset failed"; return NUHTC_E_HIP; }
  return 0;
}

static int attn_pool_route(const nuhtc_engine* e, int HW, int route) {
  return route != NUHTC_AP_AUTO ? route : e->cfg.att_pool_fp16 ? NUHTC_AP_FP16 : HW % 32 == 0 ? NUHTC_AP_GEMM : NUHTC_AP_KERNEL;
}
static int attn_pool_table(nuhtc_engine* e, const float* F, float* G, int B, int HW, float tau, int route, float* inv, float* S, float* Ft, hipStream_t s) {
  route = attn_pool_route(e, HW, route);
  if (route == NUHTC_AP_FP16) {
    RUN(launch_attn_pool_fp16(F, G, B, HW, tau, s));
  } else if (route == NUHTC_AP_GEMM) {
    if (HW % 32 != 0) FAIL(e, NUHTC_E_INVALID, "attention pool: the GEMM route needs HW % 32 == 0");
    RUN(launch_rownorm_inv(F, inv, B * HW, 64, s));
    GemmParams p1 = gp(F, F, nullptr, S, HW, HW, 64);
    p1.act = ACT_COS; p1.cos_ri = inv; p1.cos_rj = inv; p1.cos_tau = tau;
    p1.batch = B; p1.sA = (long long)HW * 64; p1.sW = (long long)HW * 64; p1.sC = (long long)HW * HW; p1.sRi = HW; p1.sRj = HW;
    RUN(egemm(e, p1, s));
    RUN(launch_transpose(F, Ft, B, HW, 64, s));
    GemmParams p2 = gp(S, Ft, nullptr, G, HW, 64, HW);
    p2.alpha = 1.0f / (float)HW;
    p2.batch = B; p2.sA = (long long)HW * HW; p2.sW = (long long)HW * 64; p2.sC = (long long)HW * 64;
    RUN(egemm(e, p2, s));
  } else if (route == NUHTC_AP_KERNEL) {
    RUN(launch_attn_pool(F, G, B, HW, tau, s));
  } else FAIL(e, NUHTC_E_INVALID, "attention pool: unknown route");
  return 0;
}

static void roi_feat_modes(RoiFeatParams& fp, float* big_part) {
  static const int& stream_few = dev_knob_ref("STREAM_FEW", 1);
  static const int& big_split = dev_knob_ref("BIG_SPLIT", 1);
  fp.stream_few = stream_few;
  fp.big_part = big_split ? big_part : nullptr; fp.big_split_max = BIG_SPLIT_MAX;
}

int run_roi_path(nuhtc_engine* e, int B, const float* rois_fixed, int n_rois, int n_dets, hipStream_t s, const nuhtc_dets* out) {
  const nuhtc_config& c = e->cfg;
  RoiWs* w = e->rw;
  const int Hn = e->Hn, Wn = e->Wn;
  const bool fixed = rois_fixed != nullptr;
  if (!out || !out->boxes || !out->labels || !out->counts) FAIL(e, NUHTC_E_INVALID, "nuhtc_dets.boxes/labels/counts are required");
  if (hipMemsetAsync(e->overflow, 0, 16, s) != hipSuccess) FAIL(e, NUHTC_E_HIP, "hipMemsetAsync failed");

  if (!fixed) {
    RpnLevels lv;
    for (int l = 0; l < 4; ++l) { lv.out[l] = e->rpn[l]; lv.h[l] = e->st[l].H; lv.w[l] = e->st[l].W; lv.stride[l] = 4 << l; }
    RpnSelParams sp;
    sp.nms_pre = c.rpn_nms_pre; sp.slot = w->rpn_slot; sp.cand_boxes = w->cand_boxes; sp.cand_scores = w->cand_scores; sp.cand_count = w->cand_count; sp.keys = w->rpn_keys; sp.key_stride = w->rpn_key_stride;
    sp.img_h = e->Hv; sp.img_w = e->Wv; sp.min_size = c.rpn_min_bbox_size;
    hipStream_t s2 = e->cfg.schedule == NUHTC_SCHED_THROUGHPUT ? s : e->side;
    if (s2 != s && hipStreamWaitEvent(s2, e->ev_rpn, 0) != hipSuccess) FAIL(e, NUHTC_E_HIP, "hipStreamWaitEvent failed");
    RUN(launch_rpn_select(lv, sp, B, s2));
    NmsParams np;
    memset(&np, 0, sizeof(np));
    np.boxes = w->cand_boxes; np.scores = w->cand_scores; np.ids = nullptr; np.group_count = w->cand_count; np.n_groups = 4; np.slot = w->rpn_slot;
    np.cap = w->rpn_cap; np.cap_pow2 = w->rpn_pow2; np.iou_thr = c.rpn_nms_iou; np.max_keep = c.rpn_max_per_img;
    np.sorted_boxes = w->nms_sboxes; np.sorted_src = w->nms_src; np.n_total = w->nms_ntotal; np.mask = w->nms_mask;
    np.out_dets = w->rpn_dets; np.out_src = w->rpn_src; np.out_counts = w->rpn_counts;
    np.seg_start = w->nms_seg_start; np.seg_n = w->nms_seg_n; np.sorted_pos = w->nms_pos; np.keepbits = w->nms_keepbits;
    RUN(launch_nms_levels(np, B, s2));
    if (s2 != s && hipEventRecord(e->ev_side, s2) != hipSuccess) FAIL(e, NUHTC_E_HIP, "hipEventRecord failed");
    if (c.watershed_proposal && c.max_cc_proposals > 0) {
      CcParams cp;
      cp.sem_pred = e->sem_pred; cp.h = e->st[0].H; cp.w = e->st[0].W; cp.img_h = e->Hv; cp.img_w = e->Wv; cp.min_area = 10;    cp.cap = c.max_cc_proposals;
      cp.mask_a = w->cc_a; cp.mask_b = w->cc_b; cp.touch = w->cc_touch; cp.labels = w->cc_labels; cp.stats = w->cc_stats; cp.boxes = w->cc_boxes;
      cp.counts = w->cc_counts; cp.overflow = e->overflow; cp.list = w->cc_list; cp.nlist = w->cc_nlist;
      RUN(launch_cc_proposals(cp, B, s));
    }
  }
  const bool use_cc = !fixed && c.watershed_proposal && c.max_cc_proposals > 0;
  for (int l = 2; l < 4; ++l)
    RUN(attn_pool_table(e, e->x[l], l == 2 ? w->G2 : w->G3, B, e->st[l].H * e->st[l].W, c.att_thres, NUHTC_AP_AUTO, w->ap_inv, w->ap_S, w->ap_Ft, s));
  if (e->cfg.schedule != NUHTC_SCHED_THROUGHPUT && hipStreamWaitEvent(s, fixed ? e->ev_rpn : e->ev_side, 0) != hipSuccess) FAIL(e, NUHTC_E_HIP, "hipStreamWaitEvent failed");
  RUN(launch_build_rois(use_cc ? w->cc_boxes : nullptr, w->cc_counts, std::max(c.max_cc_proposals, 1), w->rpn_dets, w->rpn_counts, c.rpn_max_per_img,
                        rois_fixed, n_rois, w->rois, w->roi_off, w->roi_cnt, w->roi_total, B, s));
  const int Rcap = fixed ? B * n_rois : B * e->roi_cap;

  RoiFeatParams fp;
  fp.rois = w->rois; fp.r_dev = w->roi_total; fp.x0 = e->x[0]; fp.x1 = e->x[1]; fp.G2 = w->G2; fp.G3 = w->G3; fp.sem = e->sem_feat; fp.x0sem = e->x0sem;
  fp.H0 = e->st[0].H; fp.W0 = e->st[0].W; fp.H1 = e->st[1].H; fp.W1 = e->st[1].W; fp.H2 = e->st[2].H; fp.W2 = e->st[2].W; fp.H3 = e->st[3].H; fp.W3 = e->st[3].W;
  fp.out = w->feats; fp.fb_count = w->fb_count; fp.fb_list = w->fb_list; fp.list_cap = w->total_cap; fp.mid_list = w->mid_list; fp.fb_flag = w->fb_flag;
  roi_feat_modes(fp, w->big_part);
  for (int k = 0; k < 3; ++k) {
    auto it = e->bufs.find("rois_stage" + std::to_string(k));
    if (it != e->bufs.end() && e->debug_tokens)
      if (hipMemcpyAsync(it->second.ptr, w->rois, (size_t)Rcap * 5 * sizeof(float), hipMemcpyDeviceToDevice, s) != hipSuccess) FAIL(e, NUHTC_E_HIP, "memcpy failed");
    RUN(launch_roi_feat(fp, 7, Rcap, s, e->cfg.schedule == NUHTC_SCHED_THROUGHPUT ? nullptr : e->side, e->ev_fpn, e->ev_side, e->side2, e->ev_side2));
    {
      GemmParams p = gp(w->feats, e->fc1_w[k], e->fc1_b[k], w->h1, Rcap, 256, 3136);
      p.act = ACT_RELU; p.m_dev = w->roi_total;
      RUN(egemm(e, p, s));
    }
    {
      GemmParams p = gp(w->h1, e->fc2_w[k], e->fc2_b[k], w->h2, Rcap, 256, 256);
      p.act = ACT_RELU; p.m_dev = w->roi_total;
      RUN(egemm(e, p, s));
    }
    BboxTailParams tp;
    tp.h = w->h2; tp.w = e->head_w[k]; tp.b = e->head_b[k]; tp.nc = c.num_classes; tp.r_dev = w->roi_total; tp.cls = w->cls[k]; tp.reg = w->reg[k];
    tp.refine = k < 2; tp.rois = w->rois;
    for (int j = 0; j < 4; ++j) tp.stds[j] = c.stage_stds[k][j];
    tp.img_w = (float)e->Wv; tp.img_h = (float)e->Hv;
    RUN(launch_bbox_tail(tp, Rcap, s));
  }
  DetCandParams dp;
  dp.rois = w->rois; dp.cls0 = w->cls[0]; dp.cls1 = w->cls[1]; dp.cls2 = w->cls[2]; dp.reg2 = w->reg[2]; dp.roi_off = w->roi_off; dp.roi_cnt = w->roi_cnt;
  dp.nc = c.num_classes;
  for (int j = 0; j < 4; ++j) dp.stds[j] = c.stage_stds[2][j];
  dp.img_w = (float)e->Wv; dp.img_h = (float)e->Hv; dp.scale = c.scale_factor; dp.score_thr = fixed ? -1.0f : c.score_thr;
  dp.cand_boxes = w->dc_boxes; dp.cand_scores = w->dc_scores; dp.cand_ids = w->dc_ids; dp.cand_count = w->dc_count; dp.cap = w->det_cap;
  RUN(launch_det_candidates(dp, B, s));
  {
    NmsParams np;
    memset(&np, 0, sizeof(np));
    np.boxes = w->dc_boxes; np.scores = w->dc_scores; np.ids = w->dc_ids; np.group_count = w->dc_count; np.n_groups = 1; np.slot = w->det_cap;
    np.cap = w->det_cap; np.cap_pow2 = w->det_pow2; np.iou_thr = fixed ? 2.0f : c.nms_iou; np.max_keep = c.max_per_img;
    np.sorted_boxes = w->nms_sboxes; np.sorted_src = w->nms_src; np.n_total = w->nms_ntotal; np.mask = w->nms_mask;
    np.out_dets = out->boxes; np.out_src = w->det_src; np.out_counts = out->counts;
    RUN(launch_nms(np, B, s));
  }
  DetFinishParams df;
  df.B = B; df.max_keep = c.max_per_img; df.dets = out->boxes; df.keep_src = w->det_src; df.cand_ids = w->dc_ids; df.det_counts = out->counts;
  df.labels = out->labels; df.mask_rois = w->mask_rois; df.det_off = w->det_off; df.det_total = w->det_total; df.scale = c.scale_factor;
  df.limit = fixed ? n_dets : c.max_per_img;
  RUN(launch_det_finish(df, s));
  if (!out->masks) return 0;

  const int Dcap = B * c.max_per_img;
  RoiFeatParams mp = fp;
  mp.rois = w->mask_rois; mp.r_dev = w->det_total; mp.out = w->mfeat;
  RUN(launch_roi_feat(mp, 14, Dcap, s));
  float* a = w->mfeat;
  float* b = w->mtmpA;
  for (int j = 0; j < 4; ++j) {
    GemmParams p = gp(a, e->mk_w[j], e->mk_b[j], b, Dcap * 196, 64, 576);
    p.amode = A_CONV3; p.cH = 14; p.cW = 14; p.cC = 64; p.act = ACT_RELU; p.m_dev = w->det_total; p.m_mul = 196;
    RUN(egemm(e, p, s));
    a = b;
    b = (b == w->mtmpA) ? w->mtmpB : w->mtmpA;
  }
  {
    GemmParams p = gp(a, e->mk_up_w, e->mk_up_b, w->mup, Dcap * 196, 256, 64);
    p.act = ACT_RELU; p.store = ST_DECONV2; p.cH = 14; p.cW = 14; p.ldc = 64; p.m_dev = w->det_total; p.m_mul = 196;
    RUN(egemm(e, p, s));
  }
  RUN(launch_conv1x1_n1_dev(w->mup, e->mk_lw, e->mk_lb, w->mprob, Dcap * 784, w->det_total, 784, 1, s));
  PasteParams pp;
  pp.prob = w->mprob; pp.mask_rois = w->mask_rois; pp.det_off = w->det_off; pp.det_counts = out->counts; pp.max_keep = c.max_per_img;
  pp.H = c.tile_h; pp.W = c.tile_w; pp.vH = e->vh; pp.vW = e->vw; pp.scale = c.scale_factor; pp.thr = c.mask_thr_binary; pp.masks = out->masks; pp.areas = out->areas;
  RUN(launch_paste(pp, B, s));
  if (out->keep && out->areas) {
    TilePostParams tp;
    tp.dets = out->boxes; tp.labels = out->labels; tp.areas = out->areas; tp.det_counts = out->counts; tp.masks = out->masks; tp.keep = out->keep;
    tp.max_keep = c.max_per_img; tp.H = c.tile_h; tp.W = c.tile_w; tp.vH = e->vh; tp.vW = e->vw; tp.margin = c.margin; tp.min_area = c.min_area;
    tp.thr = mask_nms_thr(c.mask_nms_thr);
    RUN(launch_tile_post(tp, B, s));
  }
  return 0;
}

int nuhtc_op_roi_align(nuhtc_engine* e, const float* feat, int N, int H, int W, const float* rois, int R, int P, float scale, int sr, float* out,
                       void* stream) {
  if (!e || !feat || !rois || !out) return NUHTC_E_INVALID;
  HIP_CHECK(e, hipSetDevice(e->device));
  int rc = launch_roi_align(feat, N, H, W, 64, rois, R, nullptr, P, scale, sr, out, 0, (hipStream_t)stream);
  if (rc) FAIL(e, rc, "roi_align launch failed");
  return 0;
}

int nuhtc_op_nms(nuhtc_engine* e, const float* boxes, const float* scores, int n, float iou_thr, int32_t* keep_idx, int32_t* count_dev, void* stream) {
  if (!e || !boxes || !scores || !keep_idx || !count_dev) return NUHTC_E_INVALID;
  if (!e->finalized) FAIL(e, NUHTC_E_STATE, "nuhtc_op_nms before finalize");
  if (n < 0 || n > NMS_MAX_CAP) FAIL(e, NUHTC_E_INVALID, "nms op: n out of range");
  HIP_CHECK(e, hipSetDevice(e->device));
  hipStream_t s = (hipStream_t)stream;
  const int cap = std::max(round_up(n, 64), 64);
  DevScratch sc;
  NmsParams np;
  memset(&np, 0, sizeof(np));
  np.boxes = boxes; np.scores = scores; np.ids = nullptr; np.group_count = sc.upload(&n, 1); np.n_groups = 1; np.slot = cap; np.cap = cap; np.cap_pow2 = pow2_ge(std::max(n, 2));
  np.iou_thr = iou_thr; np.max_keep = cap; np.sorted_boxes = sc.alloc<float>((size_t)cap * 16); np.sorted_src = sc.alloc<int>((size_t)cap * 4);
  np.n_total = sc.alloc<int>(4); np.mask = sc.alloc<unsigned long long>((size_t)cap * (cap / 64) * 8); np.out_dets = sc.alloc<float>((size_t)cap * 20);
  np.out_src = keep_idx; np.out_counts = count_dev;
  if (!sc.ok()) FAIL(e, NUHTC_E_HIP, "nms op: scratch allocation failed");
  const int rc = launch_nms(np, 1, s);
  return op_finish(e, rc, s, "nms launch failed", "nms kernel failed");
}

int nuhtc_op_cc_mask(nuhtc_engine* e, const float* sem_pred, int B, int h, int w, int H, int W, uint8_t* mask_out, void* stream) {
  if (!e || !sem_pred || !mask_out) return NUHTC_E_INVALID;
  if (B < 1 || h < 1 || w < 1 || H < 2 || W < 2 || (long long)H * W > (1ll << 26)) FAIL(e, NUHTC_E_INVALID, "cc_mask op: size out of range");
  HIP_CHECK(e, hipSetDevice(e->device));
  CcParams cp;
  memset(&cp, 0, sizeof(cp));
  cp.sem_pred = sem_pred; cp.h = h; cp.w = w; cp.img_h = H; cp.img_w = W; cp.mask_a = mask_out;
  int rc = launch_cc_mask(cp, B, (hipStream_t)stream);
  if (rc) FAIL(e, rc, "cc_mask launch failed");
  return 0;
}

int nuhtc_op_cc_proposals(nuhtc_engine* e, const uint8_t* mask, int B, int H, int W, int open, int min_area, int cap, uint8_t* opened_out,
                          uint8_t* filled_out, int32_t* labels_out, int32_t* stats_out, float* boxes_out, int32_t* counts_out,
                          int32_t* overflow_out, void* stream) {
  if (!e || !mask || !opened_out || !filled_out || !labels_out || !stats_out || !boxes_out || !counts_out || !overflow_out) return NUHTC_E_INVALID;
  if (B < 1 || H < 1 || W < 1 || (long long)H * W > (1ll << 26) || cap < 1 || cap > CC_LIST_CAP)
    FAIL(e, NUHTC_E_INVALID, "cc_proposals op: size out of range");
  HIP_CHECK(e, hipSetDevice(e->device));
  hipStream_t s = (hipStream_t)stream;
  const size_t total = (size_t)B * H * W;
  DevScratch sc;
  CcParams cp;
  memset(&cp, 0, sizeof(cp));
  cp.img_h = H; cp.img_w = W; cp.min_area = min_area; cp.cap = cap;
  cp.mask_a = opened_out; cp.mask_b = filled_out; cp.touch = sc.alloc<unsigned char>(total); cp.labels = labels_out; cp.stats = stats_out;
  cp.list = sc.alloc<int>((size_t)B * CC_LIST_CAP * sizeof(int)); cp.nlist = sc.alloc<int>((size_t)B * sizeof(int));
  cp.boxes = boxes_out; cp.counts = counts_out; cp.overflow = overflow_out;
  if (!sc.ok()) FAIL(e, NUHTC_E_HIP, "cc_proposals op: scratch allocation failed");
  int rc = 0;
  if (hipMemcpyAsync(opened_out, mask, total, hipMemcpyDeviceToDevice, s) != hipSuccess || hipMemsetAsync(overflow_out, 0, sizeof(int32_t), s) != hipSuccess)
    rc = NUHTC_E_HIP;
  if (!rc) rc = launch_cc_from_mask(cp, B, open != 0, s);
  return op_finish(e, rc, s, "cc_proposals launch failed", "cc_proposals kernel failed");
}

static bool read_ints(const int32_t* dev, int n, std::vector<int>& out, hipStream_t s) {
  out.resize(n);
  return hipStreamSynchronize(s) == hipSuccess && hipMemcpy(out.data(), dev, (size_t)n * sizeof(int), hipMemcpyDeviceToHost) == hipSuccess;
}

// ... 257 lines not shown
```

nuhtc_amd/engine.py:

```python
import ctypes
import os
import sys

import numpy as np
import torch

from . import hip, nuclei, ringfeat


class HipError(RuntimeError):
    pass


class _DevView:

    def __init__(self, ptr, shape, typestr):
        self.__cuda_array_interface__ = dict(shape=tuple(int(s) for s in shape), typestr=typestr, data=(int(ptr), False),
                                             version=2, strides=None)


_TYPESTR = {0: '<f4', 1: '<i4', 2: '|u1', 3: '<u4'}
_TORCH = {0: torch.float32, 1: torch.int32, 2: torch.uint8, 3: torch.int32}


# ... 492 lines not shown
        if wn1 is not None and outn1 is None:
            outn1 = new(nimg, H, W)
        more = list(more)
        if more_out2 is None:
            more_out2 = [new(nimg, m.shape[1], m.shape[2], N2 or 32) for m in more]
        a = hip.Conv3Args(inp=x.data_ptr(), out=dp(out), w=vp(wh), bias=vp(bh), nimg=nimg, H=H, W=W, act=int(act),
                          nimg_dev=dp(nimg_dev), pipe=hip.PIPE_FP32 if pipe == 'fp32' else hip.PIPE_BF16_SPLIT, N2=int(N2), w2=vp(w2h),
                          b2=vp(b2h), act2=int(act2), store_out=int(store_out), out2=dp(out2), res2=dp(res2), out3=dp(out3), wn1=vp(wn1h),
                          bn1=vp(bn1h), outn1=dp(outn1), n_more=len(more))
        for k, m in enumerate(more[:3]):
            a.more_in[k], a.more_out2[k], a.more_H[k], a.more_W[k] = m.data_ptr(), more_out2[k].data_ptr(), m.shape[1], m.shape[2]
        self._check(self.lib.nuhtc_op_conv3(self.h, ctypes.byref(a), self._stream()))
        return dict(out=out, out2=out2, out3=out3, outn1=outn1, more_out2=more_out2)

    def op_window_msa(self, x, ln_g, ln_b, qkv_w, qkv_b, rel_table, shifted, pipe='split', order='token', out=None):
        B, H, W, C = x.shape
        h = lambda t: np.ascontiguousarray(t.detach().cpu().numpy() if isinstance(t, torch.Tensor) else t, dtype=np.float32)
        vp = lambda a: a.ctypes.data_as(ctypes.c_void_p)
        arrs = [h(t) for t in (ln_g, ln_b, qkv_w, qkv_b, rel_table)]
        want = [(C,), (C,), (3 * C, C), (3 * C,), (169, C // 32)]
        if [a.shape for a in arrs] != want:
            raise ValueError(f'op_window_msa: weight shapes {[a.shape for a in arrs]}, expected {want}')
        if out is None:
            out = torch.empty(B * H * W, C, dtype=torch.float32, device=self.device)
        a = hip.WmsaArgs(x=x.data_ptr(), out=out.data_ptr(), ln_g=vp(arrs[0]), ln_b=vp(arrs[1]), qkv_w=vp(arrs[2]), qkv_b=vp(arrs[3]),
                         rel_table=vp(arrs[4]), B=B, H=H, W=W, C=C, shifted=int(bool(shifted)),
                         pipe=hip.PIPE_FP32 if pipe == 'fp32' else hip.PIPE_BF16_SPLIT,
                         out_order=hip.ORDER_COMPACT if order == 'compact' else hip.ORDER_TOKEN)
        self._check(self.lib.nuhtc_op_window_msa(self.h, ctypes.byref(a), self._stream()))
        return out

    def op_patch_embed(self, tiles, valid_hw, scale, channel_mode, mean, std, w, b, ln_g, ln_b, want_img=True):
        B, th, tw, _ = tiles.shape
        h = lambda t: np.ascontiguousarray(t.detach().cpu().numpy() if isinstance(t, torch.Tensor) else t, dtype=np.float32)
        vp = lambda a: a.ctypes.data_as(ctypes.c_void_p)
        wh, bh, gh, lbh = h(w), h(b), h(ln_g), h(ln_b)
        if wh.shape != (96, 3, 4, 4) or bh.shape != (96,) or gh.shape != (96,) or lbh.shape != (96,) or tiles.dtype != torch.uint8:
            raise ValueError('op_patch_embed: uint8 tiles, w (96, 3, 4, 4), b / ln_g / ln_b (96,)')
        Hv, Wv = int(valid_hw[0] * float(scale) + 0.5), int(valid_hw[1] * float(scale) + 0.5)
        Hn, Wn = -(-Hv // 32) * 32, -(-Wv // 32) * 32
        tok = torch.empty(B * (Hn // 4) * (Wn // 4), 96, dtype=torch.float32, device=self.device)
        img = torch.empty(B, Hn, Wn, 3, dtype=torch.float32, device=self.device) if want_img else None
        f3 = lambda v: (ctypes.c_float * 3)(*[float(x) for x in v])
        self._check(self.lib.nuhtc_op_patch_embed(self.h, tiles.data_ptr(), B, th, tw, int(valid_hw[0]), int(valid_hw[1]), float(scale), int(channel_mode),
                                                  f3(mean), f3(std), vp(wh), vp(bh), vp(gh), vp(lbh), tok.data_ptr(),
                                                  img.data_ptr() if img is not None else None, self._stream()))
        return tok, img

    def op_layernorm(self, x, g, b, out=None):
        rows, C = x.shape
        if out is None:
            out = torch.empty_like(x)
        self._check(self.lib.nuhtc_op_layernorm(self.h, x.data_ptr(), g.data_ptr(), b.data_ptr(), out.data_ptr(), rows, C, self._stream()))
        return out

    def op_merge_ln(self, x, g, b, out=None):
        B, H, W, C = x.shape
        if out is None:
            out = torch.empty(B * (H // 2) * (W // 2), 4 * C, dtype=torch.float32, device=self.device)
        self._check(self.lib.nuhtc_op_merge_ln(self.h, x.data_ptr(), g.data_ptr(), b.data_ptr(), out.data_ptr(), B, H, W, C, self._stream()))
        return out

    def op_fpn_lateral(self, x, w, bias, ln_g=None, ln_b=None, parent=None):
        B, H, W, C = x.shape
        h = lambda t: np.ascontiguousarray(t.detach().cpu().numpy(), dtype=np.float32) if t is not None else None
        vp = lambda a: a.ctypes.data_as(ctypes.c_void_p) if a is not None else None
        wh, bh, gh, lbh = h(w), h(bias), h(ln_g), h(ln_b)
        out = torch.empty(B, H, W, 64, dtype=torch.float32, device=self.device)
        self._check(self.lib.nuhtc_op_fpn_lateral(self.h, x.data_ptr(), B, H, W, C, vp(wh), vp(bh), vp(gh), vp(lbh),
                                                  parent.data_ptr() if parent is not None else None, out.data_ptr(), self._stream()))
        return out

    def op_sem_fuse(self, g0, g1, g2, g3):
        B, H, W, _ = g0.shape
        out = torch.empty_like(g0)
        self._check(self.lib.nuhtc_op_sem_fuse(self.h, g0.data_ptr(), g1.data_ptr(), g2.data_ptr(), g3.data_ptr(), out.data_ptr(), B, H, W, self._stream()))
        return out

    def op_pointwise64(self, x, w, b, out, rows_dev=None, rows_mul=1, sigmoid=False):
        self._check(self.lib.nuhtc_op_pointwise64(self.h, x.data_ptr(), w.data_ptr(), b.data_ptr(), out.data_ptr(), x.shape[0],
                                                  rows_dev.data_ptr() if rows_dev is not None else None, int(rows_mul), int(bool(sigmoid)), self._stream()))
        return out

    def op_fpn_mean_pool(self, maps):
        B = maps[0].shape[0]
        ptrs = (ctypes.c_void_p * 4)(*[m.data_ptr() for m in maps])
        hw = (ctypes.c_int32 * 4)(*[int(m.shape[1]) for m in maps])
        feat = torch.empty(B, 256, dtype=torch.float32, device=self.device)
        self._check(self.lib.nuhtc_op_fpn_mean_pool(self.h, ptrs, hw, B, feat.data_ptr(), self._stream()))
        return feat

    def _i32(self, v):
        return v if isinstance(v, torch.Tensor) else torch.tensor(np.atleast_1d(np.asarray(v)), dtype=torch.int32, device=self.device)

    def op_bbox_tail(self, h, cls_w, cls_b, reg_w, reg_b, rois, r, stds, img_hw, refine, cls=None, reg=None):
        f = lambda t: np.ascontiguousarray(t.detach().cpu().numpy() if isinstance(t, torch.Tensor) else t, dtype=np.float32)
        vp = lambda a: a.ctypes.data_as(ctypes.c_void_p)
        cw, cb, rw, rb = f(cls_w), f(cls_b), f(reg_w), f(reg_b)
        nc, cap = cw.shape[0] - 2, h.shape[0]
        if cw.shape != (nc + 2, 256) or cb.shape != (nc + 2,) or rw.shape != (4, 256) or rb.shape != (4,):
            raise ValueError('op_bbox_tail: fc_cls (nc + 2, 256) / (nc + 2,), fc_reg (4, 256) / (4,) expected')
        if cls is None:
            cls = torch.empty(cap, 16, dtype=torch.float32, device=self.device)
        if reg is None:
            reg = torch.empty(cap, 4, dtype=torch.float32, device=self.device)
        r_dev = self._i32(r)
        a = hip.BboxTailArgs(h=h.data_ptr(), cls_w=vp(cw), cls_b=vp(cb), reg_w=vp(rw), reg_b=vp(rb), nc=nc, cap=cap, refine=int(bool(refine)),
                             stds=(ctypes.c_float * 4)(*[float(v) for v in stds]), img_w=float(img_hw[1]), img_h=float(img_hw[0]),
                             r_dev=r_dev.data_ptr(), rois=rois.data_ptr(), cls=cls.data_ptr(), reg=reg.data_ptr())
        self._check(self.lib.nuhtc_op_bbox_tail(self.h, ctypes.byref(a), self._stream()))
        return cls, reg

    def op_det_post(self, rois, cls, reg2, roi_off, roi_cnt, nc, stds, img_hw, scale, score_thr, nms_iou, max_per_img, limit=None, cap=None):
        off, cnt = self._i32(roi_off), self._i32(roi_cnt)
        B = int(cnt.shape[0])
        if cap is None:
            cap = max(64, -(-int(cnt.max().item()) * nc // 64) * 64)
        K = int(max_per_img)
        dev = dict(dtype=torch.int32, device=self.device)
        fl = dict(dtype=torch.float32, device=self.device)
        r = dict(dets=torch.zeros(B, K, 5, **fl), labels=torch.zeros(B, K, **dev), counts=torch.zeros(B, **dev), mask_rois=torch.zeros(B * K, 5, **fl),
                 det_off=torch.zeros(B, **dev), det_total=torch.zeros(1, **dev), cand_count=torch.zeros(B, **dev),
                 cand_scores=torch.zeros(B, cap, **fl), cand_ids=torch.zeros(B, cap, **dev), cand_boxes=torch.zeros(B, cap, 4, **fl))
        a = hip.DetPostArgs(rois=rois.data_ptr(), cls0=cls[0].data_ptr(), cls1=cls[1].data_ptr(), cls2=cls[2].data_ptr(), reg2=reg2.data_ptr(),
                            roi_off=off.data_ptr(), roi_cnt=cnt.data_ptr(), B=B, nc=int(nc), total=int(rois.shape[0]), cap=int(cap),
                            stds=(ctypes.c_float * 4)(*[float(v) for v in stds]), img_w=float(img_hw[1]), img_h=float(img_hw[0]),
                            scale=float(scale), score_thr=float(score_thr), nms_iou=float(nms_iou), max_per_img=K,
                            limit=K if limit is None else int(limit), **{k: v.data_ptr() for k, v in r.items()})
        self._check(self.lib.nuhtc_op_det_post(self.h, ctypes.byref(a), self._stream()))
        return r

    def op_paste(self, prob, mask_rois, det_off, det_counts, max_keep, H, W, vH, vW, scale, thr=0.5, masks=None, areas=None):
        off, cnt = self._i32(det_off), self._i32(det_counts)
        B = int(cnt.shape[0])
        if masks is None:
            masks = torch.zeros(B, max_keep, H, W // 32, dtype=torch.int32, device=self.device)
        if areas is None:
            areas = torch.zeros(B, max_keep, dtype=torch.int32, device=self.device)
        a = hip.PasteArgs(prob=prob.data_ptr(), mask_rois=mask_rois.data_ptr(), det_off=off.data_ptr(), det_counts=cnt.data_ptr(), B=B,
                          D=int(prob.shape[0]), max_keep=int(max_keep), H=int(H), W=int(W), vH=int(vH), vW=int(vW), scale=float(scale),
                          thr=float(thr), masks=masks.data_ptr(), areas=areas.data_ptr())
        self._check(self.lib.nuhtc_op_paste(self.h, ctypes.byref(a), self._stream()))
        return masks, areas

    def op_tile_post(self, dets, labels, areas, det_counts, masks, H, W, vH, vW, margin=2, min_area=10, thr=0.05, keep=None):
        cnt = self._i32(det_counts)
        B, K = int(dets.shape[0]), int(dets.shape[1])
        if keep is None:
            keep = torch.zeros(B, K, dtype=torch.uint8, device=self.device)
        a = hip.TilePostArgs(dets=dets.data_ptr(), labels=labels.data_ptr(), areas=areas.data_ptr(), det_counts=cnt.data_ptr(),
                             masks=masks.data_ptr(), keep=keep.data_ptr(), B=B, max_keep=K, H=int(H), W=int(W), vH=int(vH), vW=int(vW),
                             margin=int(margin), min_area=int(min_area), thr=float(thr))
        self._check(self.lib.nuhtc_op_tile_post(self.h, ctypes.byref(a), self._stream()))
        return keep

    def op_rpn_select(self, maps, nms_pre, img_hw, min_size, cand_boxes=None, cand_scores=None, cand_count=None):
        if len(maps) != 4 or any(m.dim() != 4 or m.shape[3] != 32 or m.shape[0] != maps[0].shape[0] or m.dtype != torch.float32 for m in maps):
            raise ValueError('op_rpn_select: four float32 maps (B, h, w, 32) expected')
        maps = [m.contiguous() for m in maps]
        B, K = int(maps[0].shape[0]), int(nms_pre)
        fl = dict(dtype=torch.float32, device=self.device)
        Ka = max(K, 1)
        if cand_boxes is None:
            cand_boxes = torch.zeros(B, 4, Ka, 4, **fl)
        if cand_scores is None:
            cand_scores = torch.zeros(B, 4, Ka, **fl)
# ... 354 lines not shown
```

nuhtc_amd/hip.py:

```python
import ctypes
import os

HERE = os.path.dirname(os.path.abspath(__file__))
LIB_PATH = os.path.join(HERE, 'libnuhtc_hip.so')

RLE_MAX_RUNS = 15360
ABI_VERSION = 12

OK, E_INVALID, E_HIP, E_STATE, E_CAPACITY, E_NOTFOUND = 0, -1, -2, -3, -4, -5
CH_AS_IS, CH_SWAP = 0, 1
OVERLAP_MASK, OVERLAP_POLYGON = 0, 1
PIPE_BF16_SPLIT, PIPE_FP32 = 0, 1
ORDER_TOKEN, ORDER_COMPACT = 0, 1
SCHED_LATENCY, SCHED_THROUGHPUT = 0, 1
EVAL_PANNUKE, EVAL_CONIC = 0, 1
TISSUE_ALL, TISSUE_MEDIAN, TISSUE_THRESHOLD = 0, 1, 2


class Config(ctypes.Structure):
    _fields_ = [
        ('abi_version', ctypes.c_int32), ('num_classes', ctypes.c_int32),
        ('tile_h', ctypes.c_int32), ('tile_w', ctypes.c_int32), ('valid_h', ctypes.c_int32), ('valid_w', ctypes.c_int32), ('max_batch', ctypes.c_int32),
        ('scale_factor', ctypes.c_float), ('mean', ctypes.c_float * 3), ('std', ctypes.c_float * 3),
        ('rpn_nms_pre', ctypes.c_int32), ('rpn_max_per_img', ctypes.c_int32),
# ... 37 lines not shown
        ('stds', ctypes.c_float * 4), ('img_w', ctypes.c_float), ('img_h', ctypes.c_float),
        ('r_dev', ctypes.c_void_p), ('rois', ctypes.c_void_p), ('cls', ctypes.c_void_p), ('reg', ctypes.c_void_p),
    ]


class DetPostArgs(ctypes.Structure):
    _fields_ = [
        ('rois', ctypes.c_void_p), ('cls0', ctypes.c_void_p), ('cls1', ctypes.c_void_p), ('cls2', ctypes.c_void_p), ('reg2', ctypes.c_void_p),
        ('roi_off', ctypes.c_void_p), ('roi_cnt', ctypes.c_void_p),
        ('B', ctypes.c_int32), ('nc', ctypes.c_int32), ('total', ctypes.c_int32), ('cap', ctypes.c_int32),
        ('stds', ctypes.c_float * 4), ('img_w', ctypes.c_float), ('img_h', ctypes.c_float), ('scale', ctypes.c_float),
        ('score_thr', ctypes.c_float), ('nms_iou', ctypes.c_float), ('max_per_img', ctypes.c_int32), ('limit', ctypes.c_int32),
        ('dets', ctypes.c_void_p), ('labels', ctypes.c_void_p), ('counts', ctypes.c_void_p), ('mask_rois', ctypes.c_void_p),
        ('det_off', ctypes.c_void_p), ('det_total', ctypes.c_void_p),
        ('cand_count', ctypes.c_void_p), ('cand_scores', ctypes.c_void_p), ('cand_ids', ctypes.c_void_p), ('cand_boxes', ctypes.c_void_p),
    ]


class PasteArgs(ctypes.Structure):
    _fields_ = [
        ('prob', ctypes.c_void_p), ('mask_rois', ctypes.c_void_p), ('det_off', ctypes.c_void_p), ('det_counts', ctypes.c_void_p),
        ('B', ctypes.c_int32), ('D', ctypes.c_int32), ('max_keep', ctypes.c_int32), ('H', ctypes.c_int32), ('W', ctypes.c_int32),
        ('vH', ctypes.c_int32), ('vW', ctypes.c_int32), ('scale', ctypes.c_float), ('thr', ctypes.c_float),
        ('masks', ctypes.c_void_p), ('areas', ctypes.c_void_p),
    ]


class TilePostArgs(ctypes.Structure):
    _fields_ = [
        ('dets', ctypes.c_void_p), ('labels', ctypes.c_void_p), ('areas', ctypes.c_void_p), ('det_counts', ctypes.c_void_p),
        ('masks', ctypes.c_void_p), ('keep', ctypes.c_void_p),
        ('B', ctypes.c_int32), ('max_keep', ctypes.c_int32), ('H', ctypes.c_int32), ('W', ctypes.c_int32), ('vH', ctypes.c_int32),
        ('vW', ctypes.c_int32), ('margin', ctypes.c_int32), ('min_area', ctypes.c_int32), ('thr', ctypes.c_float),
    ]


class RoiFeatsArgs(ctypes.Structure):
    _fields_ = [
        ('x0', ctypes.c_void_p), ('x1', ctypes.c_void_p), ('sem', ctypes.c_void_p), ('x0sem', ctypes.c_void_p), ('G2', ctypes.c_void_p),
        ('G3', ctypes.c_void_p), ('rois', ctypes.c_void_p), ('r_dev', ctypes.c_void_p),
        ('B', ctypes.c_int32), ('cap', ctypes.c_int32), ('P', ctypes.c_int32), ('H', ctypes.c_int32 * 4), ('W', ctypes.c_int32 * 4),
        ('out', ctypes.c_void_p), ('fb_flag', ctypes.c_void_p), ('counts', ctypes.c_void_p),
    ]


AP_ROUTES = {'auto': 0, 'gemm': 1, 'kernel': 2, 'fp16': 3}


class EvalArgs(ctypes.Structure):
    _fields_ = [
        ('gt_maps', ctypes.c_void_p), ('t_cap', ctypes.c_int32), ('trip_cap', ctypes.c_int32), ('joint_cap', ctypes.c_int32), ('format', ctypes.c_int32),
        ('fg_thr', ctypes.c_float), ('mask_nms_thr', ctypes.c_double),
        ('sel', ctypes.c_void_p), ('nsel', ctypes.c_void_p), ('sel_labels', ctypes.c_void_p), ('area_t', ctypes.c_void_p), ('area_p', ctypes.c_void_p),
        ('trips', ctypes.c_void_p), ('joint', ctypes.c_void_p), ('counters', ctypes.c_void_p), ('pred_maps', ctypes.c_void_p),
    ]


class StitchStore(ctypes.Structure):
    _fields_ = [
        ('n_img', ctypes.c_int32), ('cand_cap', ctypes.c_int32), ('pool_cap', ctypes.c_int32), ('work_cap', ctypes.c_int32),
        ('box', ctypes.c_void_p), ('area', ctypes.c_void_p), ('score', ctypes.c_void_p), ('label', ctypes.c_void_p), ('key', ctypes.c_void_p),
        ('off', ctypes.c_void_p), ('pool', ctypes.c_void_p), ('counters', ctypes.c_void_p), ('work', ctypes.c_void_p),
    ]


class Dets(ctypes.Structure):
    _fields_ = [('boxes', ctypes.c_void_p), ('labels', ctypes.c_void_p), ('counts', ctypes.c_void_p),
                ('masks', ctypes.c_void_p), ('areas', ctypes.c_void_p), ('keep', ctypes.c_void_p)]


EXPORTS = ['nuhtc_default_config', 'nuhtc_create', 'nuhtc_destroy', 'nuhtc_last_error', 'nuhtc_load_weight',
           'nuhtc_finalize', 'nuhtc_infer', 'nuhtc_infer_fixed_load', 'nuhtc_check', 'nuhtc_get_buffer',
           'nuhtc_op_gemm', 'nuhtc_op_gemm_split', 'nuhtc_op_roi_align', 'nuhtc_op_nms', 'nuhtc_profile_enable', 'nuhtc_profile_read', 'nuhtc_dev_knob', 'nuhtc_export_crops',
           'nuhtc_mask_contours', 'nuhtc_merge_overlap', 'nuhtc_export_kept', 'nuhtc_clock_probe', 'nuhtc_op_swin_mlp', 'nuhtc_stream', 'nuhtc_op_swin_proj_mlp', 'nuhtc_bind_host_thread',
           'nuhtc_bind_host_thread_pci', 'nuhtc_bind_host_thread_at', 'nuhtc_restore_host_thread', 'nuhtc_op_ln_gemm', 'nuhtc_op_gemm_ln_gemm', 'nuhtc_op_merge_ln_gemm', 'nuhtc_write_ring_features',
           'nuhtc_write_point_features', 'nuhtc_join_features', 'nuhtc_fill_rings', 'nuhtc_features', 'nuhtc_op_cc_mask', 'nuhtc_op_cc_proposals',
           'nuhtc_op_conv3', 'nuhtc_op_window_msa', 'nuhtc_op_bbox_tail', 'nuhtc_op_det_post', 'nuhtc_op_paste', 'nuhtc_op_tile_post',
           'nuhtc_op_rpn_select', 'nuhtc_op_nms_levels', 'nuhtc_op_build_rois', 'nuhtc_op_attn_pool', 'nuhtc_op_roi_feats',
           'nuhtc_eval_batch', 'nuhtc_op_eval_select', 'nuhtc_op_eval_pairs', 'nuhtc_op_eval_render', 'nuhtc_op_eval_joint',
           'nuhtc_stitch_gather', 'nuhtc_stitch_pairs', 'nuhtc_stitch_render', 'nuhtc_op_stitch_gather', 'nuhtc_op_stitch_pairs', 'nuhtc_op_stitch_render',
           'nuhtc_tissue_mask', 'nuhtc_points_polygon_test', 'nuhtc_grid_in_contour', 'nuhtc_rle_encode',
           'nuhtc_nucleus_features', 'nuhtc_op_nucleus_pool', 'nuhtc_cell_graph', 'nuhtc_nucleus_morph', 'nuhtc_op_nucleus_morph',
           'nuhtc_nucleus_texture', 'nuhtc_op_nucleus_texture', 'nuhtc_op_nucleus_gradient', 'nuhtc_op_nucleus_shape', 'nuhtc_op_ring_fill', 'nuhtc_op_frame_gather', 'nuhtc_op_ring_fsd',
           'nuhtc_op_patch_embed', 'nuhtc_op_layernorm', 'nuhtc_op_merge_ln', 'nuhtc_op_fpn_lateral', 'nuhtc_op_sem_fuse', 'nuhtc_op_pointwise64',
           'nuhtc_op_fpn_mean_pool', 'nuhtc_cell_spatial', 'nuhtc_cell_clusters', 'nuhtc_cell_mst', 'nuhtc_cell_proximity', 'nuhtc_cell_density', 'nuhtc_cell_regions', 'nuhtc_cell_margin',
           'nuhtc_cell_enrichment', 'nuhtc_enrichment_permutation', 'nuhtc_cell_territory']

_lib = None


def load():
    global _lib
    if _lib is not None:
        return _lib
    if not os.path.exists(LIB_PATH):
        raise ImportError(f'{LIB_PATH} not found: the HIP extension is required (no CPU fallback exists). '
                          'Build it with `python -m nuhtc_amd.build` (hipcc, --offload-arch=gfx950).')
    import torch
    lib = ctypes.CDLL(LIB_PATH)
    vp, ci, cf = ctypes.c_void_p, ctypes.c_int, ctypes.c_float
    lib.nuhtc_default_config.argtypes = [ctypes.POINTER(Config)]
    lib.nuhtc_default_config.restype = None
    lib.nuhtc_create.argtypes = [ctypes.POINTER(Config), ci, ctypes.POINTER(vp)]
    lib.nuhtc_destroy.argtypes = [vp]
    lib.nuhtc_destroy.restype = None
    lib.nuhtc_last_error.argtypes = [vp]
    lib.nuhtc_last_error.restype = ctypes.c_char_p
    lib.nuhtc_load_weight.argtypes = [vp, ctypes.c_char_p, vp, ctypes.POINTER(ctypes.c_int64), ci]
    lib.nuhtc_finalize.argtypes = [vp]
    lib.nuhtc_infer.argtypes = [vp, vp, ci, ci, vp, ctypes.POINTER(Dets)]
    lib.nuhtc_features.argtypes = [vp, vp, ci, ci, vp, vp]
    lib.nuhtc_infer_fixed_load.argtypes = [vp, vp, ci, ci, vp, ci, ci, vp, ctypes.POINTER(Dets)]
    lib.nuhtc_check.argtypes = [vp, vp]
    lib.nuhtc_get_buffer.argtypes = [vp, ctypes.c_char_p, ctypes.POINTER(vp), ctypes.POINTER(ctypes.c_int64),
                                     ctypes.POINTER(ci), ctypes.POINTER(ci)]
    lib.nuhtc_op_gemm.argtypes = [vp, vp, vp, vp, vp, ci, ci, ci, ci, vp]
    lib.nuhtc_op_gemm_split.argtypes = [vp, vp, vp, vp, vp, vp, ci, ci, ci, ci, vp]
    lib.nuhtc_op_ln_gemm.argtypes = [vp, vp, ci, vp, vp, vp, vp, vp, vp, ci, ci, ci, ci, vp]
    lib.nuhtc_op_gemm_ln_gemm.argtypes = [vp, vp, vp, vp, vp, vp, vp, vp, vp, vp, vp, vp, ci, ci, ci, ci, ci, vp]
    lib.nuhtc_op_merge_ln_gemm.argtypes = [vp, vp, ci, ci, ci, ci, vp, vp, vp, vp, vp]
    lib.nuhtc_op_swin_mlp.argtypes = [vp, vp, vp, vp, vp, vp, vp, vp, vp, ci, ci, vp]
    lib.nuhtc_op_swin_proj_mlp.argtypes = [vp, vp, vp, vp, vp, vp, vp, vp, vp, vp, vp, vp, ci, ci, vp]
    lib.nuhtc_op_roi_align.argtypes = [vp, vp, ci, ci, ci, vp, ci, ci, cf, ci, vp, vp]
    lib.nuhtc_op_nms.argtypes = [vp, vp, vp, ci, cf, vp, vp, vp]
    lib.nuhtc_op_cc_mask.argtypes = [vp, vp, ci, ci, ci, ci, ci, vp, vp]
    lib.nuhtc_op_cc_proposals.argtypes = [vp, vp, ci, ci, ci, ci, ci, ci, vp, vp, vp, vp, vp, vp, vp, vp]
    lib.nuhtc_op_conv3.argtypes = [vp, ctypes.POINTER(Conv3Args), vp]
    lib.nuhtc_op_window_msa.argtypes = [vp, ctypes.POINTER(WmsaArgs), vp]
    f3 = ctypes.POINTER(cf)
    lib.nuhtc_op_patch_embed.argtypes = [vp, vp, ci, ci, ci, ci, ci, cf, ci, f3, f3, vp, vp, vp, vp, vp, vp, vp]
    lib.nuhtc_op_layernorm.argtypes = [vp, vp, vp, vp, vp, ci, ci, vp]
    lib.nuhtc_op_merge_ln.argtypes = [vp, vp, vp, vp, vp, ci, ci, ci, ci, vp]
    lib.nuhtc_op_fpn_lateral.argtypes = [vp, vp, ci, ci, ci, ci, vp, vp, vp, vp, vp, vp, vp]
    lib.nuhtc_op_sem_fuse.argtypes = [vp, vp, vp, vp, vp, vp, ci, ci, ci, vp]
    lib.nuhtc_op_pointwise64.argtypes = [vp, vp, vp, vp, vp, ci, vp, ci, ci, vp]
    lib.nuhtc_op_fpn_mean_pool.argtypes = [vp, ctypes.POINTER(vp), ctypes.POINTER(ctypes.c_int32), ci, vp, vp]
    lib.nuhtc_op_bbox_tail.argtypes = [vp, ctypes.POINTER(BboxTailArgs), vp]
    lib.nuhtc_op_det_post.argtypes = [vp, ctypes.POINTER(DetPostArgs), vp]
    lib.nuhtc_op_paste.argtypes = [vp, ctypes.POINTER(PasteArgs), vp]
    lib.nuhtc_op_tile_post.argtypes = [vp, ctypes.POINTER(TilePostArgs), vp]
    i4 = ctypes.POINTER(ctypes.c_int32)
    lib.nuhtc_op_rpn_select.argtypes = [vp, ctypes.POINTER(vp), i4, i4, ci, ci, ci, ci, cf, vp, vp, vp, vp]
    lib.nuhtc_op_nms_levels.argtypes = [vp, vp, vp, vp, ci, ci, ci, cf, ci, ci, vp, vp, vp, vp]
    lib.nuhtc_op_build_rois.argtypes = [vp, vp, vp, ci, vp, vp, ci, vp, ci, ci, ci, vp, vp, vp, vp, vp]
    lib.nuhtc_op_attn_pool.argtypes = [vp, vp, ci, ci, cf, ci, vp, vp]
    lib.nuhtc_op_roi_feats.argtypes = [vp, ctypes.POINTER(RoiFeatsArgs), vp]
    lib.nuhtc_eval_batch.argtypes = [vp, ctypes.POINTER(Dets), ci, ctypes.POINTER(EvalArgs), vp]
    lib.nuhtc_op_eval_select.argtypes = [vp, vp, ci, vp, vp, vp, ci, ci, ci, ci, cf, ctypes.c_double, vp, vp, vp, vp]
    lib.nuhtc_op_eval_pairs.argtypes = [vp, vp, vp, vp, vp, ci, ci, ci, ci, ci, ci, ci, vp, vp, vp, vp, vp]
    lib.nuhtc_op_eval_render.argtypes = [vp, vp, vp, vp, vp, ci, ci, ci, ci, ci, ci, vp, vp]
    lib.nuhtc_op_eval_joint.argtypes = [vp, vp, ci, vp, ci, ci, ci, ci, ci, ci, vp, vp, vp]
    sst = ctypes.POINTER(StitchStore)
    lib.nuhtc_stitch_gather.argtypes = [vp, ctypes.POINTER(Dets), ci, vp, cf, cf, sst, vp]
    lib.nuhtc_op_stitch_gather.argtypes = [vp, vp, vp, vp, vp, vp, ci, ci, ci, ci, cf, cf, sst, vp]
    lib.nuhtc_stitch_pairs.argtypes = lib.nuhtc_op_stitch_pairs.argtypes = [vp, sst, ci, vp, ci, vp, ci, ci, ci, ci, vp, vp, vp, vp]
    lib.nuhtc_stitch_render.argtypes = lib.nuhtc_op_stitch_render.argtypes = [vp, sst, ci, vp, ci, ci, ci, vp, vp, vp, vp]
    lib.nuhtc_mask_contours.argtypes = [vp, ctypes.POINTER(Dets), ci, ci, vp, vp, vp]
    lib.nuhtc_merge_overlap.argtypes = [ci, vp, vp, vp, vp, vp, ctypes.c_int64, ctypes.c_int64, ci, ctypes.c_double, ci, ci, ci, ci, vp, vp]
    lib.nuhtc_tissue_mask.argtypes = [ci, vp, ci, ci, ctypes.c_int64, ci, ci, ci, ci, ci, ci, vp, vp, vp, vp, vp]
    lib.nuhtc_points_polygon_test.argtypes = [ci, vp, ctypes.c_int64, vp, ctypes.c_int64, vp, vp]
    lib.nuhtc_grid_in_contour.argtypes = [ci, ci, ci, ci, ci, ci, vp, ci, ci, vp, ctypes.c_int64, vp, ctypes.c_int64, vp, ci, ci, ci, vp, vp]
    lib.nuhtc_rle_encode.argtypes = [ci, vp, vp, ci, ci, ci, ci, vp, vp, vp, ctypes.c_int64, vp, vp]
    lib.nuhtc_nucleus_features.argtypes = [vp, ctypes.POINTER(Dets), ci, vp, vp, ci, vp, vp]
    lib.nuhtc_op_nucleus_pool.argtypes = [vp, ctypes.POINTER(vp), i4, i4, i4, ci, vp, ci, ci, ci, vp, vp, ci, vp, vp]
    lib.nuhtc_cell_graph.argtypes = [ci, vp, vp, ctypes.c_int64, ci, ci, ci, ci, ci, ci, ci, vp, vp, vp, vp]
    lib.nuhtc_cell_spatial.argtypes = [ci, vp, vp, ctypes.c_int64, ci, i4, ci, ci, ci, ci, ci, vp, vp, vp, vp]
    lib.nuhtc_cell_clusters.argtypes = [ci, vp, vp, ctypes.c_int64, ci, ci, ci, ci, ci, ci, ci, ci, vp, vp, vp, vp, vp, vp, vp, vp,
                                        ctypes.POINTER(ctypes.c_int64), vp]
    lib.nuhtc_cell_mst.argtypes = [ci, vp, vp, ctypes.c_int64, ci, ci, ci, ci, ci, ci, ci, vp, vp, vp] + [ctypes.POINTER(ctypes.c_int64)] * 3 + [vp]
    lib.nuhtc_cell_proximity.argtypes = [ci, vp, vp, ctypes.c_int64, ci, ci, ci, ctypes.c_int64, ci, ci, ci, ci, vp, vp, vp, vp] + [ctypes.POINTER(ctypes.c_int64)] * 2 + [vp]
    lib.nuhtc_cell_density.argtypes = [ci, vp, vp, ctypes.c_int64] + [ci] * 11 + [vp, vp, vp]
    lib.nuhtc_cell_territory.argtypes = [ci, vp, vp, ctypes.c_int64] + [ci] * 11 + [vp] * 9
    lib.nuhtc_cell_regions.argtypes = [ci, vp, vp, ctypes.c_int64, ci, vp, vp, ctypes.c_int64, ctypes.c_int64, ci, ctypes.c_int64, ci, ci, ci, ci, vp, vp, vp, vp,
                                       ctypes.POINTER(ctypes.c_int64), vp]
    lib.nuhtc_cell_margin.argtypes = [ci, vp, vp, ctypes.c_int64, ci, vp, vp, ctypes.c_int64, ctypes.c_int64, ctypes.POINTER(ctypes.c_int32), ci, ci, ctypes.c_int64,
                                      ci, ci, ci, ci, vp, vp, vp, vp, vp, ctypes.POINTER(ctypes.c_int64), vp]
    lib.nuhtc_cell_enrichment.argtypes = [ci, vp, vp, ctypes.c_int64, ci, ci, ci, ctypes.c_uint32, ci, ci, ci, ci, vp, vp, vp, vp]
    lib.nuhtc_enrichment_permutation.argtypes = [ctypes.c_int64, ctypes.c_uint32, ci, vp]
    lib.nuhtc_nucleus_morph.argtypes = [vp, ctypes.POINTER(Dets), ci, vp, ci, vp, i4, vp, vp, ci, vp, vp, vp]
    lib.nuhtc_op_nucleus_morph.argtypes = [vp, vp, ci, vp, i4, ci, vp, ci, ci, ci, vp, vp, ci, vp, vp, vp]
    lib.nuhtc_nucleus_texture.argtypes = [vp, ctypes.POINTER(Dets), ci, vp, ci, vp, i4, vp, vp, ci, vp, vp]
    lib.nuhtc_op_nucleus_texture.argtypes = [vp, vp, ci, vp, i4, ci, vp, ci, ci, ci, vp, vp, ci, vp, vp]
    lib.nuhtc_op_nucleus_gradient.argtypes = [vp, vp, ci, vp, i4, ci, vp, ci, ci, ci, vp, vp, ci, ci, vp, vp]
    lib.nuhtc_op_nucleus_shape.argtypes = [vp, ci, vp, ci, ci, ci, vp, vp, ci, vp, vp]
    lib.nuhtc_op_ring_fill.argtypes =[ci, vp, ctypes.c_int64, vp, vp, ci, ci, vp, vp, vp]
    lib.nuhtc_op_frame_gather.argtypes = [ci, vp, ci, ci, ci, ci, vp, ci, ci, vp, vp]
    lib.nuhtc_op_ring_fsd.argtypes = [ci, vp, ctypes.c_int64, vp, ci, vp, vp, vp]
    lib.nuhtc_export_kept.argtypes = [vp, ctypes.POINTER(Dets), ci, vp, vp, ci, ci, vp, vp, vp, vp, vp, vp, vp, vp]
    lib.nuhtc_export_crops.argtypes = [vp, vp, vp, ci, vp, vp, vp, vp, ci, vp]
    lib.nuhtc_profile_enable.argtypes = [ci]
    lib.nuhtc_clock_probe.argtypes = [ci, ctypes.c_uint64, vp, vp]
    lib.nuhtc_dev_knob.argtypes = [ctypes.c_char_p, ci]
    lib.nuhtc_bind_host_thread.argtypes = [ci]
    lib.nuhtc_bind_host_thread_pci.argtypes = [ctypes.c_char_p]
    lib.nuhtc_bind_host_thread_at.argtypes = [ctypes.c_char_p, ctypes.c_char_p]
    lib.nuhtc_restore_host_thread.argtypes = []
    lib.nuhtc_stream.argtypes = [vp]
    lib.nuhtc_profile_read.argtypes = [ctypes.c_char_p, ctypes.c_size_t]
    pcp = ctypes.POINTER(ctypes.c_char_p)
    lib.nuhtc_write_ring_features.argtypes = [vp, vp, vp, vp, ctypes.c_int64, ctypes.c_char_p, pcp, pcp, ctypes.c_int32, vp, ctypes.c_int64, vp, ctypes.c_int32]
    lib.nuhtc_write_point_features.argtypes = [vp, vp, vp, ctypes.c_int64, ctypes.c_char_p, pcp, pcp, ctypes.c_int32, vp, ctypes.c_int64]
    lib.nuhtc_join_features.argtypes = [vp, vp, vp, ctypes.c_int64, vp, ctypes.c_int64, ctypes.c_int32]
    lib.nuhtc_fill_rings.argtypes = [vp, vp, ctypes.c_int64, vp, vp, vp, vp, ctypes.c_int64, ctypes.c_int32]
    for name in EXPORTS:
        fn = getattr(lib, name)
        if fn.restype is ctypes.c_int or name not in ('nuhtc_default_config', 'nuhtc_destroy', 'nuhtc_last_error', 'nuhtc_stream'):
            fn.restype = ci
    lib.nuhtc_last_error.restype = ctypes.c_char_p
    lib.nuhtc_default_config.restype = None
    lib.nuhtc_destroy.restype = None
    lib.nuhtc_stream.restype = ctypes.c_void_p
    for fn in (lib.nuhtc_write_ring_features, lib.nuhtc_write_point_features, lib.nuhtc_join_features, lib.nuhtc_fill_rings):
        fn.restype = ctypes.c_int64
    _lib = lib
    return lib


def default_config():
# ... 82 lines not shown
```

Baseline: 2066.

## Fuse mask deconv GEMM with final 1x1 sigmoid conv in epilogue

The mask head's 2x2 deconvolution GEMM (ReLU, stored as a D×784×64 map) followed by a separate 1×1 N=1 conv plus sigmoid is fused. A new ST_DECONV2_DOT epilogue computes the 64-channel dot product per output tap using shuffles and writes mask probabilities directly, which removes the large intermediate write and re-read and one kernel launch. It forces a fixed NT=4 tile, is limited to the split-weight pipe, and adds an op entry point for testing.

Result: no change. 2077 (median of 6 runs) (+0.5%).

```diff
diff --git a/include/nuhtc_hip.h b/include/nuhtc_hip.h
--- a/include/nuhtc_hip.h
+++ b/include/nuhtc_hip.h
@@ -176,6 +176,9 @@
 int nuhtc_op_pointwise64(nuhtc_engine* e, const float* x_dev, const float* w_dev, const float* b_dev, float* y_dev, int rows, const int32_t* rows_dev,
                          int rows_mul, int sigmoid, void* stream);
 int nuhtc_op_fpn_mean_pool(nuhtc_engine* e, const float* const maps[4], const int32_t hw[4], int B, float* feat_dev, void* stream);
+int nuhtc_op_mask_tail(nuhtc_engine* e, const float* x_dev, const float* Wup_dev, const float* Wup_host, const float* bup_dev, const float* w1_dev,
+                       const float* b1_dev, float* out_dev, int cap, const int32_t* dets_dev, int sigmoid, const float* res_dev, float* stats_dev,
+                       void* stream);
 typedef struct nuhtc_bbox_tail_args {
   const float* h;
   const float* cls_w;
diff --git a/nuhtc_amd/csrc/common.h b/nuhtc_amd/csrc/common.h
--- a/nuhtc_amd/csrc/common.h
+++ b/nuhtc_amd/csrc/common.h
@@ -98,7 +98,7 @@
 
 enum AMode { A_PLAIN = 0, A_CONV3 = 1, A_LN = 2  };
 enum Act { ACT_NONE = 0, ACT_RELU = 1, ACT_GELU = 2, ACT_COS = 3  };
-enum StoreMode { ST_PLAIN = 0, ST_ROWMAP = 1, ST_DECONV2 = 2 };
+enum StoreMode { ST_PLAIN = 0, ST_ROWMAP = 1, ST_DECONV2 = 2, ST_DECONV2_DOT = 3 };
 
 struct Conv3Fuse {
   int N2;
@@ -157,6 +157,10 @@
   int row_fastest;
   int throughput;
   const Conv3Fuse* fuse;
+  const float* dot_w;
+  const float* dot_b;
+  float* dot_out;
+  int dot_sigmoid;
 };
 int launch_gemm(const GemmParams& p, hipStream_t s);
 int gemm_make_split(const float* w_host, int N, int K, std::vector<unsigned short>& out);
@@ -209,6 +213,13 @@
 int launch_sem_fuse(const float* g0, const float* g1, const float* g2, const float* g3, float* out, int B, int H, int W,
                     hipStream_t s);
 int launch_conv1x1_n1(const float* x, const float* w, const float* b, float* y, int rows, int C, hipStream_t s);
+__device__ __forceinline__ float n1_dot4(float x0, float x1, float x2, float x3, float w0, float w1, float w2, float w3) {
+  return fmaf(x3, w3, fmaf(x2, w2, fmaf(x0, w0, x1 * w1)));
+}
+__device__ __forceinline__ float n1_finish(float sum, float bias, int sigmoid) {
+  const float u = sum + bias;
+  return sigmoid ? 1.0f / (1.0f + expf(-u)) : u;
+}
 int launch_rownorm_inv(const float* x, float* inv, int rows, int C, hipStream_t s);
 int launch_transpose(const float* x, float* y, int batch, int rows, int cols, hipStream_t s);
 
diff --git a/nuhtc_amd/csrc/dense.hip b/nuhtc_amd/csrc/dense.hip
--- a/nuhtc_amd/csrc/dense.hip
+++ b/nuhtc_amd/csrc/dense.hip
@@ -54,12 +54,9 @@
   const long long stride = ((long long)gridDim.x * blockDim.x) >> 4;
   for (long long row = ((long long)blockIdx.x * blockDim.x + threadIdx.x) >> 4; row < rows; row += stride) {
     const float4 v = reinterpret_cast<const float4*>(x)[row * 16 + l];
-    float acc = v.x * ww.x + v.y * ww.y + v.z * ww.z + v.w * ww.w;
+    float acc = n1_dot4(v.x, v.y, v.z, v.w, ww.x, ww.y, ww.z, ww.w);
     acc += __shfl_xor(acc, 1); acc += __shfl_xor(acc, 2); acc += __shfl_xor(acc, 4); acc += __shfl_xor(acc, 8);
-    if (l == 0) {
-      const float u = acc + bias;
-      y[row] = sigmoid ? 1.0f / (1.0f + expf(-u)) : u;
-    }
+    if (l == 0) y[row] = n1_finish(acc, bias, sigmoid);
   }
 }
 
diff --git a/nuhtc_amd/csrc/engine.h b/nuhtc_amd/csrc/engine.h
--- a/nuhtc_amd/csrc/engine.h
+++ b/nuhtc_amd/csrc/engine.h
@@ -59,6 +59,7 @@
   float *sem_lw[4], *sem_lb[4], *sem_cw[4], *sem_cb[4], *sem_ew, *sem_eb, *sem_gw, *sem_gb;
   float *fc1_w[3], *fc1_b[3], *fc2_w[3], *fc2_b[3], *head_w[3], *head_b[3];
   float *mk_w[4], *mk_b[4], *mk_up_w, *mk_up_b, *mk_lw, *mk_lb;
+  const void* mk_up_split = nullptr;
 
   float *img, *tokA, *tokB, *xw, *qkv, *att, *hid;
   float* tok[4] = {};
diff --git a/nuhtc_amd/csrc/engine.hip b/nuhtc_amd/csrc/engine.hip
--- a/nuhtc_amd/csrc/engine.hip
+++ b/nuhtc_amd/csrc/engine.hip
@@ -1309,6 +1309,27 @@
   return op_finish(e, rc, s, "pointwise64 launch failed", "pointwise64 kernel failed");
 }
 
+int nuhtc_op_mask_tail(nuhtc_engine* e, const float* x_dev, const float* Wup_dev, const float* Wup_host, const float* bup_dev, const float* w1_dev,
+                       const float* b1_dev, float* out_dev, int cap, const int32_t* dets_dev, int sigmoid, const float* res_dev, float* stats_dev,
+                       void* stream) {
+  if (!e || !x_dev || !Wup_dev || !Wup_host || !bup_dev || !w1_dev || !b1_dev || !out_dev) return NUHTC_E_INVALID;
+  if (cap < 1 || (long long)cap * 784 * 64 >= (1ll << 31)) FAIL(e, NUHTC_E_INVALID, "mask_tail op: cap out of range");
+  if (e->cfg.matrix_pipe == NUHTC_PIPE_FP32) FAIL(e, NUHTC_E_INVALID, "mask_tail op: the one-launch tail exists on the split pipe only");
+  HIP_CHECK(e, hipSetDevice(e->device));
+  hipStream_t s = (hipStream_t)stream;
+  std::vector<unsigned short> split;
+  int rc = gemm_make_split(Wup_host, 256, 64, split);
+  if (rc) FAIL(e, rc, "gemm_make_split failed");
+  DevScratch sc;
+  GemmParams p = gp(x_dev, Wup_dev, bup_dev, nullptr, cap * 196, 256, 64);
+  p.act = ACT_RELU; p.store = ST_DECONV2_DOT; p.cH = 14; p.cW = 14; p.ldc = 64; p.m_dev = dets_dev; p.m_mul = 196;
+  p.Wsplit = sc.upload(split); p.dot_w = w1_dev; p.dot_b = b1_dev; p.dot_out = out_dev; p.dot_sigmoid = sigmoid ? 1 : 0;
+  p.res = res_dev; p.ldr = 256; p.stats_out = stats_dev;
+  if (!sc.ok()) FAIL(e, NUHTC_E_HIP, "mask_tail op: scratch upload failed");
+  rc = launch_gemm(p, s);
+  return op_finish(e, rc, s, "mask_tail launch refused (no residual, no statistics) or failed", "mask_tail kernel failed");
+}
+
 int nuhtc_op_fpn_mean_pool(nuhtc_engine* e, const float* const maps[4], const int32_t hw[4], int B, float* feat_dev, void* stream) {
   if (!e || !maps || !hw || !feat_dev || B < 1) return NUHTC_E_INVALID;
   PoolLevels p{};
diff --git a/nuhtc_amd/csrc/gemm.hip b/nuhtc_amd/csrc/gemm.hip
--- a/nuhtc_amd/csrc/gemm.hip
+++ b/nuhtc_amd/csrc/gemm.hip
@@ -9,7 +9,7 @@
 
 #include "split_math.h"
 
-template <int MT, int NT, int WM, int WN>
+template <int MT, int NT, int WM, int WN, bool DOT = false>
 __device__ __forceinline__ void gemm_epilogue(const GemmParams& p, f32x16 (&acc)[MT][NT], float* lds, float* __restrict__ C, int z, int m0, int n0,
                                               int Meff, const float* ln_rstd = nullptr ) {
   const int tid = threadIdx.x;
@@ -48,7 +48,7 @@
         const int y = q / p.upW, x = q - y * p.upW;
         aux[j] = (b * (p.upH >> 1) + (y >> 1)) * (p.upW >> 1) + (x >> 1);
       }
-    } else if (p.store == ST_DECONV2) {
+    } else if (DOT || p.store == ST_DECONV2) {
 #pragma unroll
       for (int j = 0; j < 4; ++j) {
         const int hw = p.cH * p.cW;
@@ -69,7 +69,7 @@
     }
     float s_piv[4] = {0.f, 0.f, 0.f, 0.f}, s_1[4] = {0.f, 0.f, 0.f, 0.f}, s_2[4] = {0.f, 0.f, 0.f, 0.f};
     const float* colp = p.act == ACT_COS ? rj : p.bias;
-    const float* rowp = p.res ? p.res : p.up;
+    const float* rowp = DOT ? nullptr : p.res ? p.res : p.up;
     const int rowld = p.res ? p.ldr : p.N;
     unsigned rowoff[4];
 #pragma unroll
@@ -79,6 +79,14 @@
     for (int t = 0; t < NT; ++t) {
       colv[t] = v4f{0.f, 0.f, 0.f, 0.f};
       if (colp) colv[t] = *reinterpret_cast<const v4f*>(colp + n0 + (wn * NT + t) * 32 + c4);
+    }
+    v4f dotw[2] = {v4f{0.f, 0.f, 0.f, 0.f}, v4f{0.f, 0.f, 0.f, 0.f}};
+    float dotb = 0.f, dpart[4] = {0.f, 0.f, 0.f, 0.f};
+    if constexpr (DOT) {
+      static_assert(NT % 2 == 0 && WN == 1, "a 64-channel tap is two column tiles of one wave");
+      dotw[0] = *reinterpret_cast<const v4f*>(p.dot_w + c4);
+      dotw[1] = *reinterpret_cast<const v4f*>(p.dot_w + 32 + c4);
+      dotb = p.dot_b[0];
     }
     v4f rowv[4];
 #define EPI_LOADS(t_)                                                                                                   \
@@ -110,7 +118,7 @@
         }
         if (rowp) v[j] += rowv[j];
       }
-      if (p.stats_out) {
+      if (!DOT && p.stats_out) {
 #pragma unroll
         for (int j = 0; j < 4; ++j) {
           if (t == 0) s_piv[j] = __shfl(v[j].x, lane & ~7);
@@ -122,6 +130,19 @@
       __builtin_amdgcn_sched_barrier(0);
       if (t + 1 < NT) EPI_LOADS(t + 1)
       __builtin_amdgcn_sched_barrier(0);
+      if constexpr (DOT) {
+        const v4f w = dotw[t & 1];
+#pragma unroll
+        for (int j = 0; j < 4; ++j) {
+          float d = n1_dot4(v[j].x, v[j].y, v[j].z, v[j].w, w.x, w.y, w.z, w.w);
+          d += __shfl_xor(d, 1); d += __shfl_xor(d, 2); d += __shfl_xor(d, 4);
+          if ((t & 1) == 0) dpart[j] = d;
+          else if ((lane & 7) == 0 && ((okmask >> j) & 1u)) {
+            const int tap = (n0 >> 6) + (t >> 1);
+            p.dot_out[(long long)aux[j] + (tap >> 1) * (2 * p.cW) + (tap & 1)] = n1_finish(dpart[j] + d, dotb, p.dot_sigmoid);
+          }
+        }
+      } else {
 #ifdef NUHTC_GEMM_NOSTORE
 #ifndef NUHTC_GEMM_NOSTORE_K
 #define NUHTC_GEMM_NOSTORE_K 0
@@ -138,9 +159,10 @@
           *reinterpret_cast<v4f*>(C + (long long)drow[j] * p.ldc + n) = v[j];
         }
       }
+      }
       __builtin_amdgcn_sched_barrier(0);
     }
-    if (p.stats_out) {
+    if (!DOT && p.stats_out) {
       constexpr float inv_n = 1.0f / (32.0f * NT * WN);
       const int ntn = p.N / (32 * NT * WN), tile_n = n0 / (32 * NT * WN);
 #pragma unroll
@@ -392,7 +414,7 @@
 #undef STAMP
 }
 
-template <int MT, int NT, int AMODE>
+template <int MT, int NT, int AMODE, bool DOT = false>
 __global__ __launch_bounds__(256, (MT * NT <= 4 ? 3 : 2)) void gemm_split_kernel(GemmParams p) {
   constexpr int WM = 4, WN = 1, BK = 16;
   constexpr int BM = 128 * MT, BN = 32 * NT;
@@ -705,7 +727,7 @@
 #undef S_AOFF
 #undef S_STORE_TILE
   STAMP(st2 = __builtin_amdgcn_s_memtime();)
-  gemm_epilogue<MT, NT, WM, WN>(p, acc, lds, C, z, m0, n0, Meff, AMODE == A_LN ? lds + LDSF : nullptr);
+  gemm_epilogue<MT, NT, WM, WN, DOT>(p, acc, lds, C, z, m0, n0, Meff, AMODE == A_LN ? lds + LDSF : nullptr);
 #ifdef NUHTC_GEMM_STAMPS
   st3 = __builtin_amdgcn_s_memtime();
   __builtin_amdgcn_s_waitcnt(0x0070);
@@ -751,14 +773,15 @@
   return 0;
 }
 
-template <int MT, int NT>
+template <int MT, int NT, bool DOT = false>
 static void launch_split(const GemmParams& q, hipStream_t s) {
   const int mtiles = cdiv(q.M, 128 * MT);
   dim3 grid(cdiv(mtiles, 8) * 8 * (q.N / (32 * NT)), 1, q.batch > 0 ? q.batch : 1);
   if (q.amode == A_LN && q.n_pad > 0) grid.x += cdiv(cdiv(q.n_pad, 64), 8) * 8;
   static const int& lds_pad = dev_knob_ref("GEMM_LDS_PAD", 0);
   const unsigned pad = (unsigned)lds_pad;
-  if (q.amode == A_CONV3) hipLaunchKernelGGL((gemm_split_kernel<MT, NT, A_CONV3>), grid, dim3(256), pad, s, q);
+  if constexpr (DOT) hipLaunchKernelGGL((gemm_split_kernel<MT, NT, A_PLAIN, true>), grid, dim3(256), pad, s, q);
+  else if (q.amode == A_CONV3) hipLaunchKernelGGL((gemm_split_kernel<MT, NT, A_CONV3>), grid, dim3(256), pad, s, q);
   else if (q.amode == A_LN) {
     if constexpr (NT == 3 || (NT == 2 && MT == 1)) hipLaunchKernelGGL((gemm_split_kernel<MT, NT, A_LN>), grid, dim3(256), pad, s, q);
   } else hipLaunchKernelGGL((gemm_split_kernel<MT, NT, A_PLAIN>), grid, dim3(256), pad, s, q);
@@ -775,6 +798,10 @@
     return NUHTC_E_INVALID;
   if (p.stats_out && (!p.Wsplit || p.N % 96 != 0 || p.batch > 1 || (p.store != ST_PLAIN && p.store != ST_ROWMAP) || p.amode == A_CONV3)) return NUHTC_E_INVALID;
   if ((p.res && (long long)p.M * p.ldr >= (1ll << 31)) || (p.up && (long long)p.M * p.N >= (1ll << 31))) return NUHTC_E_INVALID;
+  const bool dot = p.store == ST_DECONV2_DOT;
+  if (dot && (!p.Wsplit || p.N != 256 || p.ldc != 64 || !p.dot_w || !p.dot_b || !p.dot_out || p.batch > 1 || p.amode != A_PLAIN || p.res || p.up || p.stats_out || p.fuse ||
+              (p.act != ACT_NONE && p.act != ACT_RELU) || p.cH < 1 || p.cW < 1 || p.M % (p.cH * p.cW) != 0 || (long long)p.M * 4 >= (1ll << 31)))
+    return NUHTC_E_INVALID;
   GemmParams q = p;
   if (q.alpha == 0.f) q.alpha = 1.f;
   if (q.Wsplit && q.batch > 1) q.Wsplit = nullptr;
@@ -786,9 +813,9 @@
     long long mt = cdiv(p.M, 128) * (long long)(p.batch > 0 ? p.batch : 1);
     if (p.m_dev) mt = (mt + 1) / 2;
     const int limit = q.Wsplit ? sfill : fill;
-    if (!(q.Wsplit && nt == 3) && q.amode != A_LN)
+    if (!(q.Wsplit && nt == 3) && q.amode != A_LN && !dot)
       while (nt > 1 && mt * (p.N / (32 * nt)) < limit) { if (nt > 2 && p.N % 64 == 0) nt = 2; else nt = 1; }
-    if (force_nt > 0 && p.N % (32 * force_nt) == 0) nt = force_nt;
+    if (force_nt > 0 && p.N % (32 * force_nt) == 0 && !dot) nt = force_nt;
     if (q.amode == A_LN && nt != 3 && nt != 2) return NUHTC_E_INVALID;
     if (q.stats_out && nt != 3) return NUHTC_E_INVALID;
   }
@@ -803,11 +830,11 @@
   if (prof_enabled()) {
     static std::map<long long, std::string> names;
     long long key = ((long long)nt << 40) | ((long long)p.N << 20) | p.K | ((long long)(p.amode == A_CONV3) << 44) | ((long long)halo << 45) | ((long long)(p.fuse ? p.fuse->N2 / 32 : 0) << 46) | ((long long)(p.fuse ? p.fuse->n_more : 0) << 52) |
-                    ((long long)(p.amode == A_LN) << 50) | ((long long)(p.stats_out != nullptr) << 51);
+                    ((long long)(p.amode == A_LN) << 50) | ((long long)(p.stats_out != nullptr) << 51) | ((long long)dot << 56);
     auto it = names.find(key);
     if (it == names.end())
       it = names.emplace(key, "gemm_kernel<" + std::to_string(nt) + ">|N" + std::to_string(p.N) + "|K" + std::to_string(p.K) + (p.amode == A_CONV3 ? (halo ? "|conv3halo" : "|conv3") : "") + (p.fuse ? "+pw" + std::to_string(p.fuse->N2) + (p.fuse->n_more ? "x" + std::to_string(1 + p.fuse->n_more) + "maps" : "") : "") +
-                                    (p.amode == A_LN ? "|ln" : "") + (p.stats_out ? "|stats" : "")).first;
+                                    (p.amode == A_LN ? "|ln" : "") + (p.stats_out ? "|stats" : "") + (dot ? "|deconv_dot" : "")).first;
     tag = it->second.c_str();
   }
   const double row_term = p.res ? (double)p.M * p.N : p.up ? 0.25 * p.M * p.N : 0.0;
@@ -817,7 +844,7 @@
   if (p.fuse && p.fuse->n_more > 0 && p.amode == A_CONV3)
     for (int k = 0; k < p.fuse->n_more && k < 3; ++k) more_rows += (double)(p.M / (p.cH * p.cW)) * p.fuse->more_H[k] * p.fuse->more_W[k];
   const double more_flop = p.fuse ? 2.0 * more_rows * 64 * (p.K + p.fuse->N2) : 0.0, more_bytes = p.fuse ? 4.0 * more_rows * (64 + p.fuse->N2) : 0.0;
-  ProfScope ps(tag, 2.0 * p.M * p.N * p.K * nb + fuse_flop + more_flop, 4.0 * nb * ((double)p.M * p.K + (double)p.N * p.K + (double)p.M * p.N + row_term) + fuse_bytes + more_bytes, s);
+  ProfScope ps(tag, 2.0 * p.M * p.N * p.K * nb + fuse_flop + more_flop, 4.0 * nb * ((double)p.M * p.K + (double)p.N * p.K + (double)p.M * (dot ? 4 : p.N)  + row_term) + fuse_bytes + more_bytes, s);
   ps.device_rows(p.m_dev, p.m_mul, p.M);
 #ifdef NUHTC_GEMM_STAMPS
   static unsigned long long* stamp_buf = nullptr;
@@ -832,6 +859,8 @@
   if (halo) {
     const int rc = launch_conv3_split(q, s);
     if (rc) return rc;
+  } else if (dot) {
+    launch_split<1, 4, true>(q, s);
   } else if (q.Wsplit) {
     static const int& force_mt = dev_knob_ref("SPLIT_MT", 0);
     const long long blocks2 = (long long)cdiv(p.M, 256) * (p.N / (32 * nt));
diff --git a/nuhtc_amd/csrc/roi_engine.hip b/nuhtc_amd/csrc/roi_engine.hip
--- a/nuhtc_amd/csrc/roi_engine.hip
+++ b/nuhtc_amd/csrc/roi_engine.hip
@@ -96,6 +96,8 @@
     for (int t = 0; t < 4; ++t)
       for (int oc = 0; oc < 64; ++oc) b[t * 64 + oc] = ub->data[oc];
     if ((rc = upload_gemm_weight(e, &e->mk_up_w, w, 256, 64)) || (rc = upload(e, &e->mk_up_b, b)) || (rc = upload(e, &e->mk_lw, lw->data)) || (rc = upload(e, &e->mk_lb, lb->data))) return rc;
+    const auto sp = e->wsplit.find(e->mk_up_w);
+    e->mk_up_split = sp != e->wsplit.end() ? sp->second.planes : nullptr;
   }
   return 0;
 }
@@ -167,8 +169,9 @@
   const int D = w->mask_cap;
   if ((rc = ws(e, &w->mask_rois, "mask_rois", {D, 5}, 0)) || (rc = ws(e, &w->det_off, "det_off", {B}, 1)) || (rc = ws(e, &w->det_total, "det_total", {1}, 1)) ||
       (rc = ws(e, &w->mfeat, "mask_feats", {D, 196, 64}, 0)) || (rc = ws(e, &w->mtmpA, nullptr, {D, 196, 64}, 0)) || (rc = ws(e, &w->mtmpB, nullptr, {D, 196, 64}, 0)) ||
-      (rc = ws(e, &w->mup, nullptr, {D, 784, 64}, 0)) || (rc = ws(e, &w->mprob, "mask_prob", {D, 28, 28}, 0)))
+      (rc = ws(e, &w->mprob, "mask_prob", {D, 28, 28}, 0)))
     return rc;
+  if (!e->mk_up_split && (rc = ws(e, &w->mup, nullptr, {D, 784, 64}, 0))) return rc;
   if (hipMemset(e->overflow, 0, 16) != hipSuccess) { e->err = "hipMemset failed"; return NUHTC_E_HIP; }
   return 0;
 }
@@ -313,9 +316,12 @@
   {
     GemmParams p = gp(a, e->mk_up_w, e->mk_up_b, w->mup, Dcap * 196, 256, 64);
     p.act = ACT_RELU; p.store = ST_DECONV2; p.cH = 14; p.cW = 14; p.ldc = 64; p.m_dev = w->det_total; p.m_mul = 196;
+    if (e->mk_up_split) {
+      p.store = ST_DECONV2_DOT; p.Wsplit = e->mk_up_split; p.dot_w = e->mk_lw; p.dot_b = e->mk_lb; p.dot_out = w->mprob; p.dot_sigmoid = 1;
+    }
     RUN(egemm(e, p, s));
-  }
-  RUN(launch_conv1x1_n1_dev(w->mup, e->mk_lw, e->mk_lb, w->mprob, Dcap * 784, w->det_total, 784, 1, s));
+    if (!e->mk_up_split) RUN(launch_conv1x1_n1_dev(w->mup, e->mk_lw, e->mk_lb, w->mprob, Dcap * 784, w->det_total, 784, 1, s));
+  }
   PasteParams pp;
   pp.prob = w->mprob; pp.mask_rois = w->mask_rois; pp.det_off = w->det_off; pp.det_counts = out->counts; pp.max_keep = c.max_per_img;
   pp.H = c.tile_h; pp.W = c.tile_w; pp.vH = e->vh; pp.vW = e->vw; pp.scale = c.scale_factor; pp.thr = c.mask_thr_binary; pp.masks = out->masks; pp.areas = out->areas;
diff --git a/nuhtc_amd/engine.py b/nuhtc_amd/engine.py
--- a/nuhtc_amd/engine.py
+++ b/nuhtc_amd/engine.py
@@ -598,6 +598,13 @@
                                                   rows_dev.data_ptr() if rows_dev is not None else None, int(rows_mul), int(bool(sigmoid)), self._stream()))
         return out
 
+    def op_mask_tail(self, x, w_up, b_up, w1, b1, out, dets_dev=None, sigmoid=False, res=None, stats=None):
+        wh = np.ascontiguousarray(w_up.detach().cpu().numpy(), dtype=np.float32)
+        ptr = lambda t: t.data_ptr() if t is not None else None
+        self._check(self.lib.nuhtc_op_mask_tail(self.h, x.data_ptr(), w_up.data_ptr(), wh.ctypes.data_as(ctypes.c_void_p), b_up.data_ptr(), w1.data_ptr(),
+                                                b1.data_ptr(), out.data_ptr(), x.shape[0], ptr(dets_dev), int(bool(sigmoid)), ptr(res), ptr(stats), self._stream()))
+        return out
+
     def op_fpn_mean_pool(self, maps):
         B = maps[0].shape[0]
         ptrs = (ctypes.c_void_p * 4)(*[m.data_ptr() for m in maps])
diff --git a/nuhtc_amd/hip.py b/nuhtc_amd/hip.py
--- a/nuhtc_amd/hip.py
+++ b/nuhtc_amd/hip.py
@@ -143,7 +143,7 @@
            'nuhtc_tissue_mask', 'nuhtc_points_polygon_test', 'nuhtc_grid_in_contour', 'nuhtc_rle_encode',
            'nuhtc_nucleus_features', 'nuhtc_op_nucleus_pool', 'nuhtc_cell_graph', 'nuhtc_nucleus_morph', 'nuhtc_op_nucleus_morph',
            'nuhtc_nucleus_texture', 'nuhtc_op_nucleus_texture', 'nuhtc_op_nucleus_gradient', 'nuhtc_op_nucleus_shape', 'nuhtc_op_ring_fill', 'nuhtc_op_frame_gather', 'nuhtc_op_ring_fsd',
-           'nuhtc_op_patch_embed', 'nuhtc_op_layernorm', 'nuhtc_op_merge_ln', 'nuhtc_op_fpn_lateral', 'nuhtc_op_sem_fuse', 'nuhtc_op_pointwise64',
+           'nuhtc_op_patch_embed', 'nuhtc_op_layernorm', 'nuhtc_op_merge_ln', 'nuhtc_op_fpn_lateral', 'nuhtc_op_sem_fuse', 'nuhtc_op_pointwise64', 'nuhtc_op_mask_tail',
            'nuhtc_op_fpn_mean_pool', 'nuhtc_cell_spatial', 'nuhtc_cell_clusters', 'nuhtc_cell_mst', 'nuhtc_cell_proximity', 'nuhtc_cell_density', 'nuhtc_cell_regions', 'nuhtc_cell_margin',
            'nuhtc_cell_enrichment', 'nuhtc_enrichment_permutation', 'nuhtc_cell_territory']
 
@@ -195,6 +195,7 @@
     lib.nuhtc_op_fpn_lateral.argtypes = [vp, vp, ci, ci, ci, ci, vp, vp, vp, vp, vp, vp, vp]
     lib.nuhtc_op_sem_fuse.argtypes = [vp, vp, vp, vp, vp, vp, ci, ci, ci, vp]
     lib.nuhtc_op_pointwise64.argtypes = [vp, vp, vp, vp, vp, ci, vp, ci, ci, vp]
+    lib.nuhtc_op_mask_tail.argtypes = [vp, vp, vp, vp, vp, vp, vp, vp, ci, vp, ci, vp, vp, vp]
     lib.nuhtc_op_fpn_mean_pool.argtypes = [vp, ctypes.POINTER(vp), ctypes.POINTER(ctypes.c_int32), ci, vp, vp]
     lib.nuhtc_op_bbox_tail.argtypes = [vp, ctypes.POINTER(BboxTailArgs), vp]
     lib.nuhtc_op_det_post.argtypes = [vp, ctypes.POINTER(DetPostArgs), vp]
```
